# jlvdb/yet_another_wizz

Hardware: AMD Instinct MI355X
Metric: candidate pairs/s (higher is better)
Workload: dtype f64

## Files before the change

### yet_another_wizz_amd/csrc/yawhip.hip

```cpp

#include <hip/hip_runtime.h>

#include <algorithm>
#include <atomic>
#include <numeric>
#include <thread>
#include <chrono>
#include <climits>
#include <cmath>
#include <cstdarg>
#include <cstdio>
#include <cstdlib>
#include <cstring>
#include <memory>
#include <new>
#include <string>
#include <system_error>
#include <type_traits>
#include <utility>
#include <functional>
#include <vector>

#include "yawhip.h"
#include "yawhip_sort.h"

namespace {
struct Trace {
    bool on = getenv("YAWHIP_TRACE") != nullptr;
    int n = 0;
    const char *name[32];
    std::chrono::steady_clock::time_point at[32];
    void mark(const char *what) {
        if (on && n < 32) { name[n] = what; at[n++] = std::chrono::steady_clock::now(); }
    }
    void flush() {
        if (on && n > 1) {
            fprintf(stderr, "[yawhip trace]");
            for (int i = 1; i < n; ++i)
                fprintf(stderr, " %s +%.1f", name[i], std::chrono::duration<double, std::micro>(at[i] - at[i - 1]).count());
            fprintf(stderr, " | total %.1f us\n", std::chrono::duration<double, std::micro>(at[n - 1] - at[0]).count());
        }
        n = 0;
    }
};
thread_local Trace g_trace;


constexpr int WG = 256;
constexpr int STAGE = 256;
#ifndef YAW_MSTAGE
#define YAW_MSTAGE 64
#endif
#ifndef YAW_MWG
#define YAW_MWG 64
#endif
constexpr int MWG = YAW_MWG;
static_assert(MWG == 64, "the band kernels are single-wave workgroups: their lane tile is 64 * R objects");
constexpr int MSTAGE = YAW_MSTAGE;
constexpr int MAX_EDGES = 512;
constexpr int SEG_STRIPS_MIN_RUN = 16;
constexpr int BAND_MIN_STREAM_RUN = 64;
constexpr int64_t SYNC_GRID_MIN_ITEMS = 400000;
constexpr int MAX_STRIP_REACH = 12;
constexpr int COUNT_FLUSH_MASK = (1 << 13) - 1;
constexpr int MERGED_FLUSH_MASK = (1 << 16) - 1;
constexpr int SPLIT_JOBS = 1;
constexpr double PAD_COORD = 4.0;

thread_local std::string g_last_error;

int fail(int code, const char *fmt, ...) {
    char buf[1024];
    va_list ap;
    va_start(ap, fmt);
    vsnprintf(buf, sizeof buf, fmt, ap);
    va_end(ap);
    g_last_error = buf;
    return code;
}

#define HIP_TRY(expr)                                                                              \
    do {                                                                                           \
        hipError_t e_ = (expr);                                                                    \
        if (e_ != hipSuccess)                                                                      \
            return fail(e_ == hipErrorOutOfMemory ? YAWHIP_ERR_OOM : YAWHIP_ERR_HIP, "%s failed: %s (%s:%d)", \
                        #expr, hipGetErrorString(e_), __FILE__, __LINE__);                         \
    } while (0)

struct CatView {
    const double *x, *y, *z, *w;
    const int64_t *off;
    int nb;
    const double *key;
    int axis;
};

struct alignas(16) Obj {
    double x, y, z, w;
};

struct alignas(16) ObjF {
    float x, y, z, pad;
};

constexpr double FILTER_GUARD = 8.0 * 5.9604644775390625e-8;
constexpr double UNIT_NORM_TOL = 1e-9;

constexpr int MAX_WIN = 3;
struct alignas(16) Item {
    int64_t a0;
    int32_t na;
    int32_t slot;
    int32_t pot;
    int32_t nwin;
    int64_t b0[MAX_WIN];
    int32_t nb[MAX_WIN];
    int32_t pad_;
};
static_assert(sizeof(Item) == 64, "Item layout");
constexpr int SLOT_MASK = 0x3fffffff;
__host__ __device__ inline int item_slot(const Item &it) { return it.slot & SLOT_MASK; }
__host__ __device__ inline int item_orient(const Item &it) { return (int)((unsigned)it.slot >> 30); }

typedef const __attribute__((address_space(1))) double *gf64p;
typedef const __attribute__((address_space(1))) int32_t *gi32p;
typedef const __attribute__((address_space(1))) int64_t *gi64p;
#ifndef YAW_B32_PREFETCH
#define YAW_B32_PREFETCH 0
#endif
#ifndef YAW_B32_UNROLL
#define YAW_B32_UNROLL 1
#endif
#ifndef YAW_B32_PAIRS
#define YAW_B32_PAIRS 1
#endif
#ifndef YAW_B32_SHARE
#define YAW_B32_SHARE 1
#endif
#define YAW_STR_(x) #x
#define YAW_STR(x) YAW_STR_(x)
#ifndef YAW_B32_ITEM_PREFETCH
#define YAW_B32_ITEM_PREFETCH 0
#endif
#ifndef YAW_B32_AW_EARLY
#define YAW_B32_AW_EARLY 1
#endif
#ifndef YAW_B32_WAVES_W
#define YAW_B32_WAVES_W 5
#endif
#ifndef YAW_B32_WAVES_W1
#define YAW_B32_WAVES_W1 5
#endif
#ifndef YAW_B32_WAVES_BIG
#define YAW_B32_WAVES_BIG 6
#endif
#ifndef YAW_B32_WAVES_LT
#define YAW_B32_WAVES_LT 1
#endif
#ifndef YAW_B32_WAVES
#define YAW_B32_WAVES 1
#endif
typedef float f32x2 __attribute__((ext_vector_type(2)));
typedef float f32x4 __attribute__((ext_vector_type(4)));
typedef const __attribute__((address_space(1))) float *gf32p;
struct DevTab {
    gf64p x, y, z, w;
    gi32p k;
    gi64p off;
    gi64p vbase, slo, tiles;
    const struct TileRec *tile_rec;
    const struct RunGrid *grid;
    gf32p qx, qy, qz;
    gi32p idx;
    gi32p pos3;
    int32_t axis;
    int32_t pad_;
};
__device__ __forceinline__ gf64p tab_key(const DevTab &t) { return t.axis == 0 ? t.x : (t.axis == 1 ? t.y : t.z); }

struct TileRec {
    int64_t a0;
    int32_t na;
    int32_t run;
};
struct JobRec {
    int64_t t_lo;
    int64_t k_off;
    int64_t vbase1;
    int32_t n_strips1;
    int32_t o;
};
#ifndef YAW_RUN_GRID
#define YAW_RUN_GRID 64
#endif
#ifndef YAW_BUILD_BISECT
#define YAW_BUILD_BISECT 32
#endif
constexpr int RUN_GRID = YAW_RUN_GRID;
struct RunGrid {
    double inv;
    uint32_t g[RUN_GRID + 2];
};
__device__ __forceinline__ int run_cell(double key, double first, double inv) {
    const double f = (key - first) * inv;
    return f >= (double)RUN_GRID ? RUN_GRID - 1 : (f >= 1.0 ? (int)f : 0);
}
template <typename KeyT>
__global__ __launch_bounds__(256) void k_run_grid(int64_t n_runs, const int64_t *__restrict__ off, const KeyT *__restrict__ key,
                                                  RunGrid *__restrict__ grid) {
    const int64_t i = (int64_t)blockIdx.x * blockDim.x + threadIdx.x;
    const int64_t r = i / (RUN_GRID + 1);
    const int c = (int)(i - r * (RUN_GRID + 1));
    if (r >= n_runs) return;
    const int64_t b0 = off[r], b1 = off[r + 1];
    double inv = 0.0, first = 0.0;
    if (b1 > b0) {
        first = (double)key[b0];
        const double span = (double)key[b1 - 1] - first;
        inv = span > 0.0 ? (double)RUN_GRID / span : 0.0;
        if (!(inv < 1e300)) inv = 0.0;
    }
    int64_t l = b0, h = b1;
    while (l < h) {
        const int64_t m = (l + h) >> 1;
        if (run_cell((double)key[m], first, inv) < c) l = m + 1; else h = m;
    }
    grid[r].g[c] = (uint32_t)(l - b0);
    if (c == 0) { grid[r].inv = inv; grid[r].g[RUN_GRID + 1] = 0; }
}

__global__ __launch_bounds__(256) void k_merge_triples(int64_t n, int64_t n_runs, const int64_t *__restrict__ off,
                                                       const int32_t *__restrict__ run_group, const int64_t *__restrict__ vbase,
                                                       const int64_t *__restrict__ off3, const double *__restrict__ key,
                                                       const float *__restrict__ q, int64_t q_stride, const double *__restrict__ w,
                                                       float *__restrict__ q3, int64_t q3_stride, double *__restrict__ w3,
                                                       int32_t *__restrict__ idx3, int32_t *__restrict__ pos3) {
    const int64_t i = (int64_t)blockIdx.x * blockDim.x + threadIdx.x;
    if (i >= n) return;
    int64_t lo = 0, hi = n_runs;
    while (hi - lo > 1) {
        const int64_t mid = (lo + hi) >> 1;
        if (off[mid] <= i) lo = mid; else hi = mid;
    }
    const int64_t r = lo;
    const int64_t g = run_group[r], g_lo = vbase[g], g_hi = vbase[g + 1];
    const double ki = key[i];
    const float fx = q[i], fy = q[q_stride + i], fz = q[2 * q_stride + i];
    const double wi = w ? w[i] : 0.0;
    int64_t before[5];
#pragma unroll
    for (int d = -2; d <= 2; ++d) {
        const int64_t m = r + d;
        int64_t cnt = 0;
        if (d == 0) {
            cnt = i - off[r];
        } else if (m >= g_lo && m < g_hi) {
            int64_t l = off[m], h = off[m + 1];
            const int64_t base = l;
            if (d < 0) { while (l < h) { const int64_t mid = (l + h) >> 1; if (key[mid] <= ki) l = mid + 1; else h = mid; } }
            else       { while (l < h) { const int64_t mid = (l + h) >> 1; if (key[mid] < ki) l = mid + 1; else h = mid; } }
            cnt = l - base;
        }
        before[d + 2] = cnt;
    }
#pragma unroll
    for (int d = -1; d <= 1; ++d) {
        const int64_t t = r + d + 1 + 2 * g;
        const int64_t dst = off3[t] + before[d + 1] + before[d + 2] + before[d + 3];
        q3[dst] = fx; q3[q3_stride + dst] = fy; q3[2 * q3_stride + dst] = fz;
        idx3[dst] = (int32_t)i;
        if (w3) w3[dst] = wi;
        if (d == 0) pos3[i] = (int32_t)dst;
    }
}

constexpr int EVAL_SLOTS = 256;
constexpr int BUILD_WG = 1024;
#ifndef YAW_BUILD_WG_SMALL
#define YAW_BUILD_WG_SMALL 256
#endif
inline int build_wg_for(int64_t n_pot) { return n_pot / 256 <= 4096 ? YAW_BUILD_WG_SMALL : BUILD_WG; }
constexpr int BUILD_PREFIX_LDS = 1024;

constexpr int ITEM_SEGS = 8;
__host__ __device__ constexpr int ITEM_SEG_CTR(int seg) { return 12 + 8 * seg; }
__device__ __forceinline__ void append_items(bool keep, const Item &it, unsigned long long work, Item *__restrict__ items,
                                             unsigned long long *__restrict__ counters, unsigned char *__restrict__ kept,
                                             unsigned long long seg_cap = 0) {
    if (keep && kept) kept[it.pot] = 1;
    __shared__ unsigned int s_cnt[BUILD_WG / 64];
    __shared__ unsigned long long s_work[BUILD_WG / 64], s_base;
    const unsigned long long mask = __builtin_amdgcn_ballot_w64(keep);
    const int lane = threadIdx.x & 63, wave = threadIdx.x >> 6;
    for (int off = 32; off > 0; off >>= 1) work += __shfl_down(work, off, 64);
    if (lane == 0) {
        s_cnt[wave] = (unsigned int)__popcll(mask);
        s_work[wave] = work;
    }
    __syncthreads();
    if (threadIdx.x == 0) {
        unsigned int total = 0;
        unsigned long long wsum = 0;
        for (int wv = 0; wv < (int)(blockDim.x >> 6); ++wv) {
            const unsigned int c = s_cnt[wv];
            s_cnt[wv] = total;
            total += c;
            wsum += s_work[wv];
        }
        if (seg_cap) {
            const int seg = (int)(blockIdx.x % ITEM_SEGS);
            s_base = (unsigned long long)seg * seg_cap + (total ? atomicAdd(&counters[ITEM_SEG_CTR(seg)], (unsigned long long)total) : 0ull);
        } else {
            s_base = total ? atomicAdd(&counters[0], (unsigned long long)total) : 0ull;
        }
        if (wsum) atomicAdd(&counters[10 + 8 * (blockIdx.x & (EVAL_SLOTS - 1))], wsum);
    }
    __syncthreads();
    if (keep) items[s_base + s_cnt[wave] + __popcll(mask & ((1ull << lane) - 1ull))] = it;
}

template <bool SWEEP>
__global__ __launch_bounds__(BUILD_WG) void k_build_items(CatView c1, CatView c2, const int32_t *__restrict__ jobs,
                                                     const int64_t *__restrict__ prefix, int n_slots, int n_bins,
                                                     int tile, const double *__restrict__ rwin, int64_t n_pot,
                                                     Item *__restrict__ items, unsigned long long *__restrict__ counters,
                                                     unsigned char *__restrict__ kept) {
    const int64_t pot = (int64_t)blockIdx.x * blockDim.x + threadIdx.x;
    bool keep = false;
    Item it{};
    unsigned long long work = 0;
    if (pot < n_pot) {
        int lo = 0, hi = n_slots;
        while (hi - lo > 1) {
            const int mid = (lo + hi) >> 1;
            if (prefix[mid] <= pot) lo = mid; else hi = mid;
        }
        const int slot = lo, job = slot / n_bins, k = slot - job * n_bins;
        const int p = jobs[2 * job], q = jobs[2 * job + 1];
        const int k1 = c1.nb == 1 ? 0 : k, k2 = c2.nb == 1 ? 0 : k;
        int64_t b0 = c1.off[(int64_t)p * c1.nb + k1], b1 = c1.off[(int64_t)p * c1.nb + k1 + 1];
        const int64_t a_seg1 = c2.off[(int64_t)q * c2.nb + k2 + 1];
        const int64_t a0 = c2.off[(int64_t)q * c2.nb + k2] + (pot - prefix[slot]) * (int64_t)tile;
        const int64_t a1 = a0 + tile < a_seg1 ? a0 + tile : a_seg1;
        if (SWEEP) {
            const double wlo = c2.key[a0] - rwin[k], whi = c2.key[a1 - 1] + rwin[k];
            int64_t l = b0, h = b1;
            while (l < h) {
                const int64_t m = (l + h) >> 1;
                if (c1.key[m] < wlo) l = m + 1; else h = m;
            }
            const int64_t first = l;
            h = b1;
            while (l < h) {
                const int64_t m = (l + h) >> 1;
                if (c1.key[m] <= whi) l = m + 1; else h = m;
            }
            b0 = first;
            b1 = l;
        }
        keep = b1 > b0;
        it.a0 = a0; it.b0[0] = b0; it.na = (int32_t)(a1 - a0); it.nb[0] = (int32_t)(b1 - b0); it.nwin = 1; it.slot = slot; it.pot = (int32_t)pot;
        work = keep ? (unsigned long long)it.na * (unsigned long long)it.nb[0] : 0ull;
    }
    if (SWEEP) {
        append_items(keep, it, work, items, counters, kept);
    } else {
        if (pot < n_pot) items[pot] = it;
        append_items(false, it, work, items, counters, nullptr);
        if (pot == 0) counters[0] = (unsigned long long)n_pot;
    }
}

__global__ __launch_bounds__(BUILD_WG) void k_build_items_strips(const DevTab *__restrict__ tabs, const JobRec *__restrict__ jobs,
                                                            const int64_t *__restrict__ prefix, int n_jobs, int reach,
                                                            int tile, double rwin, int swap, int triple, int64_t n_pot,
                                                            Item *__restrict__ items, unsigned long long *__restrict__ counters,
                                                            unsigned char *__restrict__ kept, unsigned long long seg_cap) {
    const int64_t pot = (int64_t)blockIdx.x * blockDim.x + threadIdx.x;
    bool keep = false;
    Item it{};
    unsigned long long work = 0;
    __shared__ int64_t s_prefix[BUILD_PREFIX_LDS];
    __shared__ DevTab s_tabs[6];
    static_assert(sizeof(DevTab) % 8 == 0, "DevTab is copied in 8-byte words");
    for (int e = threadIdx.x; e < (int)(6 * sizeof(DevTab) / 8); e += blockDim.x)
        reinterpret_cast<uint64_t *>(s_tabs)[e] = reinterpret_cast<const uint64_t *>(tabs)[e];
    const bool prefix_in_lds = n_jobs + 1 <= BUILD_PREFIX_LDS;
    if (prefix_in_lds)
        for (int e = threadIdx.x; e <= n_jobs; e += blockDim.x) s_prefix[e] = prefix[e];
    __syncthreads();
    if (pot < n_pot) {
        int lo = 0, hi = n_jobs;
        if (prefix_in_lds) {
            while (hi - lo > 1) {
                const int mid = (lo + hi) >> 1;
                if (s_prefix[mid] <= pot) lo = mid; else hi = mid;
            }
        } else {
            while (hi - lo > 1) {
                const int mid = (lo + hi) >> 1;
                if (prefix[mid] <= pot) lo = mid; else hi = mid;
            }
        }
        const int job = lo;
        const JobRec jr = jobs[job];
        const int o = jr.o & 3;
        it.pad_ = (jr.o >> 2) & 1;
#if defined(YAW_BUILD_TABS_GLOBAL)
        const DevTab &c1 = tabs[swap ? 3 + o : o], &c2 = tabs[swap ? o : 3 + o];
#else
        const DevTab &c1 = s_tabs[swap ? 3 + o : o], &c2 = s_tabs[swap ? o : 3 + o];
#endif
        const gf64p key1d = tab_key(c1), key2 = tab_key(c2);
        const gf32p key1f = c1.axis == 0 ? c1.qx : (c1.axis == 1 ? c1.qy : c1.qz);
        auto key1 = [&](int64_t i) { return triple ? (double)key1f[i] : key1d[i]; };
        const int nd = 2 * reach + 1, ng = (nd + MAX_WIN - 1) / MAX_WIN;
        const int64_t local = pot - (prefix_in_lds ? s_prefix[job] : prefix[job]);
        const uint32_t local32 = (uint32_t)local, tl = ng == 1 ? local32 : local32 / (uint32_t)ng;
        const int g = (int)(local32 - tl * (uint32_t)ng);
        const TileRec tr = c2.tile_rec[jr.t_lo + tl];
        const int64_t r2 = tr.run, a0 = tr.a0, a1 = a0 + tr.na;
        const double kpad = triple ? 1.2e-7 : 0.0;
        const double wlo = key2[a0] - (it.pad_ ? 0.0 : rwin) - kpad, whi = key2[a1 - 1] + rwin + kpad;
        it.a0 = a0; it.na = tr.na; it.nwin = 0;
        it.slot = (int32_t)((unsigned)job | ((unsigned)o << 30)); it.pot = (int32_t)pot;
        int64_t wb[MAX_WIN];
        uint32_t sl[MAX_WIN], sh[MAX_WIN], ul[MAX_WIN], uh[MAX_WIN];
        int32_t wn[MAX_WIN];
#pragma unroll
        for (int j = 0; j < MAX_WIN; ++j) {
            const int dd = g * MAX_WIN + j;
            const int64_t s1 = r2 + jr.k_off + (dd - reach);
            const bool valid = dd < nd && s1 >= 0 && s1 < jr.n_strips1;
            const int64_t r1 = jr.vbase1 + (valid ? s1 : 0);
            int64_t b0 = 0, b1 = 0;
            if (valid) { b0 = c1.off[r1]; b1 = c1.off[r1 + 1]; }
            const bool some = b1 > b0;
            double kfirst = 0.0, klast = 0.0;
            if (some) { kfirst = key1(b0); klast = key1(b1 - 1); }
            const bool live = some && !(klast < wlo || kfirst > whi);
            uint32_t l0 = 0, l1 = 0, u0 = 0, u1 = 0;
            if (live) {
                const double inv = c1.grid[r1].inv;
                const int cl = run_cell(wlo, kfirst, inv), cu = run_cell(whi, kfirst, inv);
                const uint32_t *gr = c1.grid[r1].g;
                l0 = gr[cl]; l1 = gr[cl + 1]; u0 = gr[cu]; u1 = gr[cu + 1];
            }
            wb[j] = b0;
            sl[j] = l0; sh[j] = l1; ul[j] = u0; uh[j] = u1;
        }
        for (int step = 0; step < YAW_BUILD_BISECT &&
                           ((sl[0] < sh[0]) | (sl[1] < sh[1]) | (sl[2] < sh[2]) | (ul[0] < uh[0]) | (ul[1] < uh[1]) | (ul[2] < uh[2])); ++step) {
            double kl[MAX_WIN], ku[MAX_WIN];
            uint32_t ml[MAX_WIN], mu[MAX_WIN];
#pragma unroll
            for (int j = 0; j < MAX_WIN; ++j) {
                ml[j] = sl[j] + ((sh[j] - sl[j]) >> 1);
                mu[j] = ul[j] + ((uh[j] - ul[j]) >> 1);
                kl[j] = ku[j] = 0.0;
                if (sl[j] < sh[j]) kl[j] = key1(wb[j] + ml[j]);
                if (ul[j] < uh[j]) ku[j] = key1(wb[j] + mu[j]);
            }
#pragma unroll
            for (int j = 0; j < MAX_WIN; ++j) {
                if (sl[j] < sh[j]) { if (kl[j] < wlo) sl[j] = ml[j] + 1; else sh[j] = ml[j]; }
                if (ul[j] < uh[j]) { if (ku[j] <= whi) ul[j] = mu[j] + 1; else uh[j] = mu[j]; }
            }
        }
#pragma unroll
        for (int j = 0; j < MAX_WIN; ++j) {
            wb[j] += sl[j];
            wn[j] = (int32_t)((YAW_BUILD_BISECT < 32 ? uh[j] : ul[j]) - sl[j]);
        }
#pragma unroll
        for (int j = 0; j < MAX_WIN; ++j) {
            if (wn[j] <= 0) continue;
            if (it.nwin == 0) { it.b0[0] = wb[j]; it.nb[0] = wn[j]; }
            else if (it.nwin == 1) { it.b0[1] = wb[j]; it.nb[1] = wn[j]; }
            else { it.b0[2] = wb[j]; it.nb[2] = wn[j]; }
            ++it.nwin;
            work += (unsigned long long)it.na * (unsigned long long)wn[j];
// ... 1026 lines not shown
            const unsigned ic = have ? (unsigned)(lane * R + r) : 0u;
            ax[r] = have ? (cl.qx + it.a0)[ic] : PAD_COORD32;
            ay[r] = have ? (cl.qy + it.a0)[ic] : PAD_COORD32;
            az[r] = have ? (cl.qz + it.a0)[ic] : PAD_COORD32;
            kb[r] = MERGED ? (have ? (cl.k + it.a0)[ic] : 0) : 0;
            aw[r] = (WEIGHTED && cl.w) ? (have ? (cl.w + it.a0)[ic] : 0.0) : (have ? 1.0 : 0.0);
        }
        float klo, khi;
        {
            const int last_r = n_own > 0 ? n_own - 1 : 0;
            float u_first = cl.axis == 0 ? ax[0] : (cl.axis == 1 ? ay[0] : az[0]), u_last = u_first;
#pragma unroll
            for (int r = 1; r < R; ++r)
                if (r == last_r) u_last = cl.axis == 0 ? ax[r] : (cl.axis == 1 ? ay[r] : az[r]);
            klo = u_first - rwin;
            khi = u_last + rwin;
        }
        unsigned int nev = 0;
        auto flush_counts = [&]() {
#if defined(YAW_FINE_DIAG) && YAW_FINE_DIAG == 5
            return;
#endif
            __syncthreads();
            for (int idx = lane; idx < nslots; idx += 64) {
                const unsigned int c = (unsigned int)hist[idx];
                hist[idx] = HistT(0);
                if (c) atomicAdd(&out_counts[(int64_t)islot * nslots + idx], (unsigned long long)c);
            }
        };
        float pm[R], pa[R];
        unsigned a_edges[R], a_rowh[R];
        const float nf_f = (float)nf;
        const unsigned a_stab = (unsigned)(size_t)(lds_byte *)reinterpret_cast<unsigned char *>(stab);
#pragma unroll
        for (int r = 0; r < R; ++r) {
            const int trow = (UNI ? 0 : (MERGED ? kb[r] : kfix)) * tw;
            pm[r] = stab[trow]; pa[r] = stab[trow + 1];
            a_edges[r] = a_stab + (unsigned)(trow + 4) * 4u;
            a_rowh[r] = a_hist + ((unsigned)(kb[r] * nf) << HB);
        }
        f32x2 ax2[R / 2 > 0 ? R / 2 : 1], ay2[R / 2 > 0 ? R / 2 : 1], az2[R / 2 > 0 ? R / 2 : 1];
        if constexpr (R >= 2) {
#pragma unroll
            for (int h = 0; h < R / 2; ++h) {
                ax2[h] = f32x2{ax[2 * h], ax[2 * h + 1]}; ay2[h] = f32x2{ay[2 * h], ay[2 * h + 1]}; az2[h] = f32x2{az[2 * h], az[2 * h + 1]};
            }
        }

        for (int win = 0; win < it.nwin; ++win) {
        if (win > 0) {
            b0 = win == 1 ? it.b0[1] : it.b0[2];
            nb_total = win == 1 ? it.nb[1] : it.nb[2];
        }
        for (int64_t st0 = 0; st0 < nb_total; st0 += CAP, ++stage_no) {
            const int n = (int)(nb_total - st0 < CAP ? nb_total - st0 : CAP);
            if (st0 > 0 || win > 0) {
                __syncthreads();
                stage_in(st0, n);
            }
            asm volatile("s_waitcnt vmcnt(0)" ::: "memory");
            __syncthreads();
            if (lane == 0) {
                stage[n] = PAD_COORD32; stage[COLB / 4 + n] = PAD_COORD32; stage[2 * (COLB / 4) + n] = PAD_COORD32;
                if (WEIGHTED) sw[n] = 0.0;
            }
            if (WEIGHTED && !cs.w)
                for (int e = lane; e < n; e += 64) sw[e] = 1.0;
            __syncthreads();
            const unsigned a_key = a_stage + COLB * (unsigned)cl.axis;
            const unsigned a_sent = a_key + ((unsigned)n << 2);
            unsigned ql = a_key - 4u, qh = ql;
            for (unsigned step = 4u << (31 - __builtin_clz(n)); step >= 4u; step >>= 1) {
                const unsigned pl = ql + step, ph = qh + step;
                const float kl = *(const __attribute__((address_space(3))) float *)(size_t)(pl < a_sent ? pl : a_sent);
                const float kh = *(const __attribute__((address_space(3))) float *)(size_t)(ph < a_sent ? ph : a_sent);
                ql = kl < klo ? pl : ql;
                qh = kh <= khi ? ph : qh;
            }
            int lo = (int)((ql + 4u - a_key) >> 2), hi = (int)((qh + 4u - a_key) >> 2);
            if (n_own == 0) lo = hi = n;
            const int len = hi - lo;
            nev += (unsigned int)(len * n_own);
#if defined(YAW_FINE_DIAG) && YAW_FINE_DIAG == 1
            const int steps = 0;
#else
            const int steps = wave_max_nonneg(len);
#endif

            unsigned cur = a_stage + ((unsigned)lo << 2);
            const unsigned last = a_stage + ((unsigned)n << 2);
            struct Entry { float x, y, z; double w; unsigned at; };
            auto fetch = [&](unsigned at) {
                Entry e;
                e.at = at < last ? at : last;
                e.x = *(const __attribute__((address_space(3))) float *)(size_t)e.at;
                e.y = *(const __attribute__((address_space(3))) float *)(size_t)(e.at + COLB);
                e.z = *(const __attribute__((address_space(3))) float *)(size_t)(e.at + 2 * COLB);
                e.w = WEIGHTED ? lds_f64(((e.at - a_stage) << 1) + a_sw) : 1.0;
                return e;
            };
            unsigned pend[R];
#pragma unroll
            for (int r = 0; r < R; ++r) pend[r] = a_dummy;
            Entry nxt = fetch(cur);
            if constexpr (WEIGHTED) asm volatile("" :: "v"(nxt.x), "v"(nxt.y), "v"(nxt.z), "v"(nxt.w));
            else asm volatile("" :: "v"(nxt.x), "v"(nxt.y), "v"(nxt.z));
            for (int s = 0; s < steps; ++s) {
                const Entry en = nxt;
                cur += 4;
                nxt = fetch(cur);
                const unsigned a16 = en.at;
                const float ex = en.x, ey = en.y, ez = en.z;
                const double ew = en.w;
                float s32[R];
                if constexpr (R >= 2) {
#pragma unroll
                    for (int h = 0; h < R / 2; ++h) {
                        const f32x2 dx = ax2[h] - ex, dy = ay2[h] - ey, dz = az2[h] - ez;
                        const f32x2 sq = __builtin_elementwise_fma(dz, dz, __builtin_elementwise_fma(dy, dy, dx * dx));
                        s32[2 * h] = sq.x; s32[2 * h + 1] = sq.y;
                    }
                } else {
                    const float dx = ax[0] - ex, dy = ay[0] - ey, dz = az[0] - ez;
                    s32[0] = __builtin_fmaf(dz, dz, __builtin_fmaf(dy, dy, dx * dx));
                }
                int jj[R];
                bool unc[R];
                unsigned long long any_unc_mask = 0ull;
                f32x2 tb[R];
#pragma unroll
                for (int r = 0; r < R; ++r) {
                    const float fr = __builtin_rintf(__builtin_fmaf(__builtin_amdgcn_logf(s32[r]), pm[r], -pa[r]));
                    jj[r] = (int)__builtin_amdgcn_fmed3f(fr, 0.0f, nf_f);
                    tb[r] = *(const __attribute__((address_space(3))) f32x2 *)(size_t)(a_edges[r] + ((unsigned)jj[r] << 3));
                }
                if constexpr (!WEIGHTED) {
#pragma unroll
                    for (int r = 0; r < R; ++r)
                        (void)__hip_atomic_fetch_add((__attribute__((address_space(3))) unsigned int *)(size_t)pend[r], 1u,
                                                     __ATOMIC_RELAXED, __HIP_MEMORY_SCOPE_WORKGROUP);
                }
#pragma unroll
                for (int r = 0; r < R; ++r) {
                    const int j = jj[r];
                    const bool below = s32[r] < tb[r].x, above = s32[r] > tb[r].y;
                    const int bin = j - (below ? 1 : 0);
                    unc[r] = !(below | above);
                    any_unc_mask |= ~(__builtin_amdgcn_ballot_w64(below) | __builtin_amdgcn_ballot_w64(above));
                    const bool hit = ((unsigned)bin < (unsigned)nf) & !unc[r];
                    const unsigned cell = a_rowh[r] + ((unsigned)bin << HB);
                    if constexpr (WEIGHTED) {
                        if (hit)
                            (void)__hip_atomic_fetch_add((__attribute__((address_space(3))) double *)(size_t)cell, aw[r] * ew,
                                                         __ATOMIC_RELAXED, __HIP_MEMORY_SCOPE_WORKGROUP);
                    } else {
                        pend[r] = hit ? cell : a_dummy;
                    }
                }
#if defined(YAW_FINE_DIAG) && YAW_FINE_DIAG == 6
                any_unc_mask = 0ull;
#endif
                if (any_unc_mask != 0ull) {
                    const unsigned eidx = (a16 - a_stage) >> 2;
#pragma unroll
                    for (int r = 0; r < R; ++r) {
                        if (unc[r] && eidx < (unsigned)n && r < n_own) {
                            const int j = jj[r];
                            const ExactEval<1> ev = band32_exact<1>(cl.x, cl.y, cl.z, it.a0 + lane * R + r, cs.x, cs.y, cs.z,
                                                                    cs.idx ? (int64_t)cs.idx[b0 + st0 + eidx] : b0 + st0 + (int64_t)eidx,
                                                                    t + (size_t)(MERGED ? kb[r] : kfix) * n_edges + j,
                                                                    counters + 9 + 8 * (ticket & (EVAL_SLOTS - 1)));
                            const int bin = ev.s <= ev.th[0] ? j - 1 : j;
                            if ((unsigned)bin < (unsigned)nf) {
                                const unsigned cell = a_rowh[r] + ((unsigned)bin << HB);
                                if constexpr (WEIGHTED)
                                    (void)__hip_atomic_fetch_add((__attribute__((address_space(3))) double *)(size_t)cell, aw[r] * ew,
                                                                 __ATOMIC_RELAXED, __HIP_MEMORY_SCOPE_WORKGROUP);
                                else
                                    (void)__hip_atomic_fetch_add((__attribute__((address_space(3))) unsigned int *)(size_t)cell, 1u,
                                                                 __ATOMIC_RELAXED, __HIP_MEMORY_SCOPE_WORKGROUP);
                            }
                        }
                    }
                }
            }
            if constexpr (!WEIGHTED) {
#pragma unroll
                for (int r = 0; r < R; ++r)
                    (void)__hip_atomic_fetch_add((__attribute__((address_space(3))) unsigned int *)(size_t)pend[r], 1u,
                                                 __ATOMIC_RELAXED, __HIP_MEMORY_SCOPE_WORKGROUP);
            }
            if (!WEIGHTED && (stage_no & flush_mask) == flush_mask) flush_counts();
        }
        }
        if constexpr (WEIGHTED) {
            __syncthreads();
            for (int idx = lane; idx < nslots; idx += 64) {
                partials[(int64_t)it.pot * nslots + idx] = (double)hist[idx];
                hist[idx] = HistT(0);
            }
        } else {
            flush_counts();
        }
        nev = wave_sum_lane63(nev);
        if (lane == 63 && nev) atomicAdd(&counters[8 + 8 * (ticket & (EVAL_SLOTS - 1))], (unsigned long long)nev);
    }
}

__global__ void k_item_work(const Item *__restrict__ items, const unsigned long long *__restrict__ counters,
                            int slots_per_job, unsigned long long *__restrict__ job_work) {
    const unsigned long long i = (unsigned long long)blockIdx.x * blockDim.x + threadIdx.x;
    if (i >= counters[0]) return;
    const Item it = items[i];
    unsigned long long streamed = 0;
    for (int w = 0; w < it.nwin; ++w) streamed += (unsigned long long)it.nb[w];
    atomicAdd(&job_work[item_slot(it) / slots_per_job], (unsigned long long)it.na * streamed);
}

constexpr int REDUCE_CHUNK = 32;
__global__ void k_reduce_chunks(const double *__restrict__ partials, const unsigned char *__restrict__ kept,
                                const int64_t *__restrict__ prefix, const int64_t *__restrict__ cprefix, int n_slots,
                                int slab, double *__restrict__ chunk_sums) {
    const int64_t idx = (int64_t)blockIdx.x * blockDim.x + threadIdx.x;
    const int64_t g = idx / slab;
    if (g >= cprefix[n_slots]) return;
    const int e = (int)(idx - g * slab);
    int lo = 0, hi = n_slots;
    while (hi - lo > 1) {
        const int mid = (lo + hi) >> 1;
        if (cprefix[mid] <= g) lo = mid; else hi = mid;
    }
    const int64_t p0 = prefix[lo] + (g - cprefix[lo]) * REDUCE_CHUNK;
    const int64_t p1 = p0 + REDUCE_CHUNK < prefix[lo + 1] ? p0 + REDUCE_CHUNK : prefix[lo + 1];
    double acc = 0.0;
    for (int64_t pot = p0; pot < p1; ++pot)
        if (!kept || kept[pot]) acc += partials[pot * slab + e];
    chunk_sums[idx] = acc;
}

__global__ void k_reduce_slots(const double *__restrict__ chunk_sums, const int64_t *__restrict__ cprefix, int n_slots,
                               int slab, double *__restrict__ out) {
    const int64_t idx = (int64_t)blockIdx.x * blockDim.x + threadIdx.x;
    if (idx >= (int64_t)n_slots * slab) return;
    const int slot = (int)(idx / slab), e = (int)(idx - (int64_t)slot * slab);
    double acc = 0.0;
    for (int64_t g = cprefix[slot]; g < cprefix[slot + 1]; ++g) acc += chunk_sums[g * slab + e];
    out[idx] = acc;
}

template <typename F>
__device__ double numpy_sum_dev(F v, int lo, int n) {
    if (n < 8) {
        double res = 0.0;
        for (int i = 0; i < n; ++i) res += v(lo + i);
        return res;
    }
    if (n <= 128) {
        double r[8];
        for (int j = 0; j < 8; ++j) r[j] = v(lo + j);
        int i = 8;
        for (; i < n - (n % 8); i += 8)
            for (int j = 0; j < 8; ++j) r[j] += v(lo + i + j);
        double res = ((r[0] + r[1]) + (r[2] + r[3])) + ((r[4] + r[5]) + (r[6] + r[7]));
        for (; i < n; ++i) res += v(lo + i);
        return res;
    }
    int n2 = n / 2;
    n2 -= n2 % 8;
    return numpy_sum_dev(v, lo, n2) + numpy_sum_dev(v, lo + n2, n - n2);
}

__global__ void k_combine_scales(const unsigned long long *__restrict__ counts, const double *__restrict__ sums, int weighted,
                                 int64_t n_jobs, int n_bins, int nf, int n_scales, const int32_t *__restrict__ slices,
                                 const double *__restrict__ factors, double *__restrict__ out) {
    const int64_t i = (int64_t)blockIdx.x * blockDim.x + threadIdx.x;
    if (i >= n_jobs * n_bins * n_scales) return;
    const int sc = (int)(i % n_scales), k = (int)((i / n_scales) % n_bins);
    const int64_t j = i / ((int64_t)n_scales * n_bins);
    const int lo = slices[2 * (k * n_scales + sc)], hi = slices[2 * (k * n_scales + sc) + 1];
    const int64_t base = (j * n_bins + k) * (int64_t)nf;
    const double *wk = factors ? factors + (int64_t)k * nf : nullptr;
    auto value = [&](int e) {
        const double v = weighted ? sums[base + e] : (double)counts[base + e];
        return wk ? v * wk[e] : v;
    };
    out[i] = hi > lo ? numpy_sum_dev(value, lo, hi - lo) : 0.0;
}

__global__ void k_scatter_rows(const double *__restrict__ in, const int32_t *__restrict__ row_index, int64_t row, int64_t n,
                               double *__restrict__ out) {
    const int64_t i = (int64_t)blockIdx.x * blockDim.x + threadIdx.x;
    if (i >= n) return;
    const int64_t r = i / row;
    out[(int64_t)row_index[r] * row + (i - r * row)] = in[i];
}

__global__ void k_counts_to_double(const unsigned long long *__restrict__ in, double *__restrict__ out, int64_t n) {
    const int64_t i = (int64_t)blockIdx.x * blockDim.x + threadIdx.x;
    if (i < n) out[i] = (double)in[i];
}

inline DevTab make_tab(const double *x, const double *y, const double *z, const double *w, const int32_t *k, const int64_t *off,
                       const int64_t *vbase, const int64_t *slo, const int64_t *tiles, const TileRec *tile_rec, const RunGrid *grid,
                       int axis, const float *q = nullptr, int64_t q_stride = 0, const int32_t *idx = nullptr) {
    return DevTab{(gf64p)x, (gf64p)y, (gf64p)z, (gf64p)w, (gi32p)k, (gi64p)off, (gi64p)vbase, (gi64p)slo, (gi64p)tiles,
                  tile_rec, grid, (gf32p)q, (gf32p)(q ? q + q_stride : nullptr), (gf32p)(q ? q + 2 * q_stride : nullptr), (gi32p)idx,
                  (gi32p)nullptr, axis, 0};
}

template <typename T>
struct DevBuf {
    T *ptr = nullptr;
    size_t cap = 0;
    hipError_t reserve(size_t n) {
        if (n <= cap) return hipSuccess;
        if (ptr) (void)hipFree(ptr);
        ptr = nullptr;
        cap = 0;
        size_t want = n + n / 4 + 64;
        hipError_t e = hipMalloc(reinterpret_cast<void **>(&ptr), want * sizeof(T));
        if (e == hipSuccess) cap = want;
        return e;
    }
    void release() {
        if (ptr) (void)hipFree(ptr);
        ptr = nullptr;
        cap = 0;
    }
};

struct Arena {
    unsigned char *h = nullptr, *d = nullptr;
    size_t cap = 0;
    hipError_t reserve(size_t n) {
        if (n <= cap) return hipSuccess;
        release();
        const size_t want = n + n / 4 + 4096;
        hipError_t e = hipHostMalloc(reinterpret_cast<void **>(&h), want, hipHostMallocPortable);
        if (e == hipSuccess) e = hipMalloc(reinterpret_cast<void **>(&d), want);
        if (e == hipSuccess) cap = want; else release();
        return e;
    }
    void release() {
        if (h) (void)hipHostFree(h);
        if (d) (void)hipFree(d);
        h = d = nullptr;
        cap = 0;
    }
};
inline size_t align16(size_t n) { return (n + 15) & ~(size_t)15; }

}

template <typename T>
struct View {
    T *ptr = nullptr;
};

struct CallBufs {
    hipEvent_t ev0 = nullptr, ev1 = nullptr, evc0 = nullptr, evc1 = nullptr, ev_done = nullptr;
    View<int32_t> d_jobs;
    View<int64_t> d_prefix;
    View<double> d_t;
    View<float> d_dthr;
    View<float> d_thr32;
    View<double> d_rwin;
    DevBuf<Item> d_items;
    View<unsigned long long> d_ctr;
    View<unsigned long long> d_counts;
    View<double> d_sums;
    DevBuf<double> d_partials;
    DevBuf<double> d_chunk_sums;
    View<int64_t> d_cprefix;
    DevBuf<unsigned char> d_kept;
    Arena out;
    Arena comb;
    View<DevTab> d_tabs;
    hipError_t make_events() {
        hipError_t e = hipSuccess;
        for (hipEvent_t *ev : {&ev0, &ev1, &evc0, &evc1, &ev_done})
            if (e == hipSuccess && !*ev) e = hipEventCreate(ev);
        return e;
    }
    void release_all() {
        d_items.release(); d_partials.release(); d_chunk_sums.release(); d_kept.release();
        out.release(); comb.release();
        for (hipEvent_t *ev : {&ev0, &ev1, &evc0, &evc1, &ev_done}) {
            if (*ev) (void)hipEventDestroy(*ev);
            *ev = nullptr;
        }
    }
};
constexpr int MAX_BATCH = 4;
constexpr size_t MAX_PLANS = 16;

namespace {
struct HostPlan;

struct CallKey {
    uint64_t c1_uid = 0, c2_uid = 0, opt_gen = 0, hash = 0;
    int32_t n_jobs = 0, n_bins = 0, n_edges = 0, kernel = 0, n_dev = 0;
    bool want_counts = false, want_sums = false, for_work = false;
    const int32_t *jobs = nullptr;
    const double *t = nullptr;
    std::vector<int32_t> own_jobs;
    std::vector<double> own_t;

    CallKey() = default;
    CallKey(const yawhip_ctx *ctx, const yawhip_catalog *c1, const yawhip_catalog *c2, int32_t n_jobs, const int32_t *jobs,
            int32_t n_bins, int32_t n_edges, const double *t, int32_t kernel, bool want_counts, bool want_sums, bool for_work,
            int32_t n_dev = 0);
    CallKey(CallKey &&) = default;
    CallKey &operator=(CallKey &&) = default;
    CallKey(const CallKey &) = delete;
    CallKey &operator=(const CallKey &) = delete;

    void keep() {
        own_jobs.assign(jobs, jobs + 2 * (size_t)n_jobs);
        own_t.assign(t, t + (size_t)n_bins * n_edges);
        jobs = own_jobs.data();
        t = own_t.data();
    }
    bool operator==(const CallKey &o) const {
        return hash == o.hash && c1_uid == o.c1_uid && c2_uid == o.c2_uid && opt_gen == o.opt_gen && n_jobs == o.n_jobs &&
               n_bins == o.n_bins && n_edges == o.n_edges && kernel == o.kernel && n_dev == o.n_dev && want_counts == o.want_counts &&
               want_sums == o.want_sums && for_work == o.for_work &&
               memcmp(jobs, o.jobs, sizeof(int32_t) * 2 * (size_t)n_jobs) == 0 &&
               memcmp(t, o.t, sizeof(double) * (size_t)n_bins * n_edges) == 0;
    }
};
}

struct yawhip_ctx : CallBufs {
    int device = 0;
    hipStream_t stream = nullptr;
    int tile_r = 0;
    int hist_copies_log2 = -1;
    int band_batch_log2 = -1;
    int band_cap = 0;
    int seg_strips = 1;
    int seg_min_run = SEG_STRIPS_MIN_RUN;
    int debug_no_hits = 0;
    int auto_orient = 1;
    int64_t slab_budget = 1ll << 30;
    int band_grid_div = 0;
    int flush_log2 = 17;
    int spin_wait = 1;
    int item_segments = 1;
    int half_bands = 1;
    int triple_runs = 1;
    int band_fp32 = 1;
    double strip_width = 0.005;
    int default_kernel = YAWHIP_KERNEL_AUTO;
    int lds_limit = 160 * 1024;
    int n_cu = 256;
    DevBuf<unsigned long long> d_jobwork;
    DevBuf<double> d_full;
    DevBuf<int32_t> d_rowidx;
    std::vector<yawhip_ctx *> peers;
    struct Plan {
        CallKey key;
        std::vector<std::vector<int32_t>> parts;
    } plan;
    yawsort::Workspace sort_ws;
    CallBufs parked[MAX_BATCH];
    int slot = 0;
    uint64_t opt_gen = 1;
    uint64_t plan_clock = 0;
    std::vector<HostPlan *> plans;
};
inline hipError_t use_slot(yawhip_ctx *ctx, int i) {
    if (i != ctx->slot) {
        std::swap(static_cast<CallBufs &>(*ctx), ctx->parked[ctx->slot]);
        std::swap(static_cast<CallBufs &>(*ctx), ctx->parked[i]);
        ctx->slot = i;
    }
    return ctx->make_events();
}


struct StripLayout {
    bool built = false;
    double *x = nullptr, *y = nullptr, *z = nullptr, *w = nullptr;
    int32_t *k = nullptr;
    float *q = nullptr;
    int64_t q_stride = 0;
    int64_t *off = nullptr;
    std::vector<int64_t> h_off;
    std::vector<int64_t> h_vbase;
    std::vector<int64_t> h_slo;
    std::vector<int64_t> h_tiles[3];
    int64_t *d_vbase = nullptr, *d_slo = nullptr, *d_tiles[3] = {nullptr, nullptr, nullptr};
    TileRec *d_tile_rec[3] = {nullptr, nullptr, nullptr};
    RunGrid *d_grid = nullptr;
    bool triples = false;
    float *q3 = nullptr;
    int64_t q3_stride = 0;
    double *w3 = nullptr;
    int32_t *idx3 = nullptr;
    int32_t *pos3 = nullptr;
    int64_t *off3 = nullptr;
    RunGrid *d_grid3 = nullptr;
    int64_t n_groups = 0;
    int64_t device_bytes = 0;
    double obj_run = 0.0;
    double same_bin = 0.0;
    void release() {
        for (void *ptr : {(void *)x, (void *)y, (void *)z, (void *)w, (void *)k, (void *)q, (void *)off, (void *)d_vbase, (void *)d_slo,
                          (void *)d_tiles[0], (void *)d_tiles[1], (void *)d_tiles[2], (void *)d_tile_rec[0], (void *)d_tile_rec[1],
                          (void *)d_tile_rec[2], (void *)d_grid, (void *)q3, (void *)w3, (void *)idx3, (void *)pos3, (void *)off3, (void *)d_grid3})
            if (ptr) (void)hipFree(ptr);
        q3 = nullptr; w3 = nullptr; idx3 = nullptr; pos3 = nullptr; off3 = nullptr; d_grid3 = nullptr; triples = false;
        x = y = z = w = nullptr; k = nullptr; q = nullptr; off = d_vbase = d_slo = nullptr;
        d_tiles[0] = d_tiles[1] = d_tiles[2] = nullptr;
        d_tile_rec[0] = d_tile_rec[1] = d_tile_rec[2] = nullptr;
        d_grid = nullptr;
        built = false;
    }
};

struct yawhip_catalog {
    yawhip_ctx *ctx = nullptr;
    uint64_t uid = 0;
    int64_t n = 0;
    int32_t n_patches = 0, nb = 1;
    double *x = nullptr, *y = nullptr, *z = nullptr, *w = nullptr;
    int64_t *off = nullptr;
    std::vector<int64_t> h_off;
    int64_t device_bytes = 0;
    bool unit_norm = true;
    int axis = 2;
    StripLayout strips[3], seg[3];
    std::vector<yawhip_catalog *> replicas;
    bool has_strips = false;
    double strip_width = 0.0;
    std::vector<double> h_box;
};

namespace {

void drop_plans(yawhip_ctx *ctx, const yawhip_catalog *c);

const double *key_of(const double *x, const double *y, const double *z, int axis) { return axis == 0 ? x : (axis == 1 ? y : z); }
CatView view_of(const yawhip_catalog *c) {
    return CatView{c->x, c->y, c->z, c->w, c->off, c->nb, key_of(c->x, c->y, c->z, c->axis), c->axis};
}

template <typename... Params, typename... Args>
hipError_t launch(void (*kern)(Params...), dim3 grid, dim3 block, size_t lds, hipStream_t stream, Args... args) {
    if (lds > 64 * 1024) {
        const hipError_t e = hipFuncSetAttribute(reinterpret_cast<const void *>(kern), hipFuncAttributeMaxDynamicSharedMemorySize, (int)lds);
        if (e != hipSuccess) return e;
    }
    hipLaunchKernelGGL(kern, grid, block, lds, stream, args...);
    return hipGetLastError();
}

template <typename... Ts, typename V, typename F>
hipError_t pick(const V &v, F &&f) {
    hipError_t e = hipErrorInvalidValue;
    (void)(((v == Ts::value) && (e = f(Ts{}), true)) || ...);
    return e;
}
template <bool B> using Bool = std::integral_constant<bool, B>;
template <int I> using Int = std::integral_constant<int, I>;
template <int R_, int CAP_> struct Stage {
    static constexpr int R = R_, CAP = CAP_;
    static constexpr std::pair<int, int> value{R_, CAP_};
};
template <bool MERGED_, bool UNI_> struct Rows {
    static constexpr bool MERGED = MERGED_, UNI = UNI_;
    static constexpr std::pair<bool, bool> value{MERGED_, UNI_};
};

__global__ __launch_bounds__(256) void k_assign_patches(int64_t n, const double *__restrict__ x, const double *__restrict__ y,
                                                       const double *__restrict__ z, int n_centers,
                                                       const double *__restrict__ centers, int32_t *__restrict__ out) {
    extern __shared__ __attribute__((aligned(16))) unsigned char lds_raw[];
    double *c = reinterpret_cast<double *>(lds_raw);
    for (int e = threadIdx.x; e < 3 * n_centers; e += blockDim.x) c[e] = centers[e];
    __syncthreads();
    const int64_t i = (int64_t)blockIdx.x * blockDim.x + threadIdx.x;
    if (i >= n) return;
    const double px = x[i], py = y[i], pz = z[i];
    double best = INFINITY;
    int best_j = -1;
    for (int j = 0; j < n_centers; ++j) {
        const double dx = px - c[3 * j], dy = py - c[3 * j + 1], dz = pz - c[3 * j + 2];
        const double xx = dx * dx;
        const double yy = dy * dy;
        const double zz = dz * dz;
        const double sxy = xx + yy;
        const double d = sxy + zz;
        if (d < best) {
            best = d;
            best_j = j;
        }
    }
    out[i] = best_j;
}

__global__ void k_gather_columns(int64_t n, const uint32_t *__restrict__ perm, const double *__restrict__ sx,
                                 const double *__restrict__ sy, const double *__restrict__ sz, const double *__restrict__ sw,
                                 double *__restrict__ dx, double *__restrict__ dy, double *__restrict__ dz, double *__restrict__ dw) {
    const int64_t i = (int64_t)blockIdx.x * blockDim.x + threadIdx.x;
    if (i >= n) return;
    const uint32_t src = perm[i];
    dx[i] = sx[src];
    dy[i] = sy[src];
    dz[i] = sz[src];
    if (sw) dw[i] = sw[src];
}

__device__ __forceinline__ int segment_of(const int64_t *__restrict__ off, int n_seg, int64_t i) {
    int lo = 0, hi = n_seg;
    while (hi - lo > 1) {
        const int mid = (lo + hi) >> 1;
        if (off[mid] <= i) lo = mid; else hi = mid;
    }
    return lo;
}

__global__ void k_gather_bins(int64_t n, const uint32_t *__restrict__ perm, const int64_t *__restrict__ off, int64_t n_seg,
                              int n_bins, int32_t *__restrict__ bins) {
    const int64_t i = (int64_t)blockIdx.x * blockDim.x + threadIdx.x;
    if (i < n) bins[i] = segment_of(off, (int)n_seg, (int64_t)perm[i]) % n_bins;
}

__global__ void k_make_q(int64_t n, const double *__restrict__ x, const double *__restrict__ y, const double *__restrict__ z,
                         int64_t stride, float *__restrict__ q) {
    const int64_t i = (int64_t)blockIdx.x * blockDim.x + threadIdx.x;
    if (i >= n) return;
    q[i] = (float)x[i];
    q[stride + i] = (float)y[i];
    q[2 * stride + i] = (float)z[i];
}

__global__ void k_same_bin_neighbours(int64_t n, const int32_t *__restrict__ bins, unsigned long long *__restrict__ out) {
    const int64_t i = (int64_t)blockIdx.x * blockDim.x + threadIdx.x;
    const bool same = i + 1 < n && bins[i] == bins[i + 1];
    const unsigned long long m = __builtin_amdgcn_ballot_w64(same);
    if ((threadIdx.x & 63) == 0 && m) atomicAdd(out, (unsigned long long)__popcll(m));
}

__global__ void k_strip_index(int64_t n, const double *__restrict__ v, double width, const int64_t *__restrict__ poff,
                              int n_patches, int32_t *__restrict__ gidx, int32_t *__restrict__ lohi) {
    const int64_t i = (int64_t)blockIdx.x * blockDim.x + threadIdx.x;
    const bool ok = i < n;
    int32_t g = 0;
    int p = -1;
    if (ok) {
        g = width > 0.0 ? (int32_t)floor((v[i] + 1.0) / width) : 0;
        gidx[i] = g;
        p = segment_of(poff, n_patches, i);
    }
    const int p0 = __builtin_amdgcn_readfirstlane(p);
    if (__builtin_amdgcn_ballot_w64(p != p0) == 0ull) {
        if (p0 < 0) return;
        int32_t lo = g, hi = g;
        for (int off = 32; off > 0; off >>= 1) {
            lo = min(lo, __shfl_xor(lo, off, 64));
            hi = max(hi, __shfl_xor(hi, off, 64));
        }
        if ((threadIdx.x & 63) == 0) {
            atomicMin(&lohi[2 * p0], lo);
            atomicMax(&lohi[2 * p0 + 1], hi);
        }
    } else if (ok) {
        atomicMin(&lohi[2 * p], g);
        atomicMax(&lohi[2 * p + 1], g);
    }
}

__global__ void k_run_of(int64_t n, const uint32_t *__restrict__ order, const int32_t *__restrict__ gidx,
                         const int64_t *__restrict__ poff, int n_patches, const int64_t *__restrict__ vbase,
                         const int64_t *__restrict__ slo, uint32_t *__restrict__ run) {
    const int64_t i = (int64_t)blockIdx.x * blockDim.x + threadIdx.x;
    if (i >= n) return;
    const uint32_t src = order[i];
    const int p = segment_of(poff, n_patches, (int64_t)src);
    run[i] = (uint32_t)(vbase[p] + (int64_t)gidx[src] - slo[p]);
}

__global__ void k_run_offsets(const uint32_t *__restrict__ run_sorted, int64_t n, int64_t n_runs, int64_t *__restrict__ moff) {
    const int64_t r = (int64_t)blockIdx.x * blockDim.x + threadIdx.x;
    if (r > n_runs) return;
    int64_t lo = 0, hi = n;
    while (lo < hi) {
        const int64_t mid = (lo + hi) >> 1;
        if ((int64_t)run_sorted[mid] < r) lo = mid + 1; else hi = mid;
    }
    moff[r] = lo;
}

__host__ __device__ inline unsigned long long sortable_of(double d) {
    unsigned long long b;
    memcpy(&b, &d, sizeof b);
    return (b >> 63) ? ~b : (b | 0x8000000000000000ull);
}
inline double double_of(unsigned long long s) {
    const unsigned long long b = (s >> 63) ? (s & 0x7fffffffffffffffull) : ~s;
    double d;
    memcpy(&d, &b, sizeof d);
    return d;
}

__global__ void k_patch_boxes(int64_t n, const double *__restrict__ x, const double *__restrict__ y, const double *__restrict__ z,
                              const int64_t *__restrict__ poff, int n_patches, unsigned long long *__restrict__ box) {
    const int64_t i = (int64_t)blockIdx.x * blockDim.x + threadIdx.x;
    const bool ok = i < n;
    double v[3] = {0.0, 0.0, 0.0};
    int p = -1;
    bool off_sphere = false;
    if (ok) {
        v[0] = x[i]; v[1] = y[i]; v[2] = z[i];
        p = segment_of(poff, n_patches, i);
        const double n2 = v[0] * v[0] + v[1] * v[1] + v[2] * v[2];
        off_sphere = !(n2 > 1.0 - UNIT_NORM_TOL && n2 < 1.0 + UNIT_NORM_TOL);
    }
    if (__builtin_amdgcn_ballot_w64(off_sphere) != 0ull && (threadIdx.x & 63) == 0) atomicAdd(&box[(size_t)6 * n_patches], 1ull);
    const int p0 = __builtin_amdgcn_readfirstlane(p);
    if (__builtin_amdgcn_ballot_w64(p != p0) == 0ull) {
        if (p0 < 0) return;
#pragma unroll
        for (int a = 0; a < 3; ++a) {
            unsigned long long lo = sortable_of(v[a]), hi = lo;
            for (int off = 32; off > 0; off >>= 1) {
                const unsigned long long l2 = __shfl_xor(lo, off, 64), h2 = __shfl_xor(hi, off, 64);
                lo = l2 < lo ? l2 : lo;
                hi = h2 > hi ? h2 : hi;
            }
            if ((threadIdx.x & 63) == 0) {
                atomicMin(&box[(size_t)6 * p0 + a], lo);
                atomicMax(&box[(size_t)6 * p0 + 3 + a], hi);
            }
        }
    } else if (ok) {
#pragma unroll
        for (int a = 0; a < 3; ++a) {
            atomicMin(&box[(size_t)6 * p + a], sortable_of(v[a]));
            atomicMax(&box[(size_t)6 * p + 3 + a], sortable_of(v[a]));
        }
    }
}

inline int64_t seg_len(const yawhip_catalog *c, int patch, int k) {
    const int kk = c->nb == 1 ? 0 : k;
    const int64_t i = (int64_t)patch * c->nb + kk;
    return c->h_off[i + 1] - c->h_off[i];
}

int build_strip_layout(yawhip_ctx *ctx, yawhip_catalog *c, int o, bool seg) {
    StripLayout &L = seg ? c->seg[o] : c->strips[o];
    if (L.built) return YAWHIP_OK;
    const int64_t n = c->n, nseg = (int64_t)c->n_patches * c->nb;
    const int n_groups = seg ? (int)nseg : c->n_patches;
    const bool want_bins = !seg && c->nb > 1;
    const double width = c->strip_width;
    const int saxis = (o + 2) % 3;
    std::vector<int64_t> h_poff((size_t)n_groups + 1);
    for (int g = 0; g <= n_groups; ++g) h_poff[(size_t)g] = seg ? c->h_off[(size_t)g] : c->h_off[(size_t)g * c->nb];
    const size_t col = (size_t)std::max<int64_t>(n, 1) * sizeof(double) + 16;
    uint32_t *perm = nullptr, *perm2 = nullptr, *run = nullptr, *run_sorted = nullptr;
    int32_t *gidx = nullptr, *lohi = nullptr;
    int64_t *poff = nullptr;
    auto bail = [&](hipError_t err, const char *what) {
        for (void *q : {(void *)perm, (void *)perm2, (void *)run, (void *)run_sorted, (void *)gidx, (void *)lohi, (void *)poff})
            if (q) (void)hipFree(q);
        if (err == hipSuccess) return (int)YAWHIP_OK;
        L.release();
        return fail(err == hipErrorOutOfMemory ? YAWHIP_ERR_OOM : YAWHIP_ERR_HIP, "strip layout (%s) failed: %s", what,
                    hipGetErrorString(err));
    };
    HIP_TRY(hipSetDevice(ctx->device));
    std::vector<int32_t> h_lohi((size_t)2 * n_groups);
    for (int g = 0; g < n_groups; ++g) { h_lohi[(size_t)2 * g] = INT32_MAX; h_lohi[(size_t)2 * g + 1] = INT32_MIN; }
    const size_t n1 = (size_t)std::max<int64_t>(n, 1);
    hipError_t e = hipMalloc(reinterpret_cast<void **>(&poff), (size_t)(n_groups + 1) * sizeof(int64_t));
    if (e == hipSuccess) e = hipMalloc(reinterpret_cast<void **>(&lohi), (size_t)2 * n_groups * sizeof(int32_t));
    if (e == hipSuccess) e = hipMalloc(reinterpret_cast<void **>(&gidx), n1 * sizeof(int32_t));
    if (e == hipSuccess) e = hipMalloc(reinterpret_cast<void **>(&perm), n1 * sizeof(uint32_t));
    if (e == hipSuccess) e = hipMalloc(reinterpret_cast<void **>(&perm2), n1 * sizeof(uint32_t));
    if (e == hipSuccess) e = hipMalloc(reinterpret_cast<void **>(&run), n1 * sizeof(uint32_t));
    if (e == hipSuccess) e = hipMalloc(reinterpret_cast<void **>(&run_sorted), n1 * sizeof(uint32_t));
    if (e == hipSuccess)
        e = hipMemcpyAsync(poff, h_poff.data(), (size_t)(n_groups + 1) * sizeof(int64_t), hipMemcpyHostToDevice, ctx->stream);
    if (e == hipSuccess)
        e = hipMemcpyAsync(lohi, h_lohi.data(), (size_t)2 * n_groups * sizeof(int32_t), hipMemcpyHostToDevice, ctx->stream);
    if (e != hipSuccess) return bail(e, "strip tables");
    const unsigned ngrid = (unsigned)((n1 + 255) / 256);
    hipLaunchKernelGGL(k_strip_index, dim3(ngrid), dim3(256), 0, ctx->stream, n, key_of(c->x, c->y, c->z, saxis), width, poff,
                       n_groups, gidx, lohi);
    e = hipMemcpyAsync(h_lohi.data(), lohi, (size_t)2 * n_groups * sizeof(int32_t), hipMemcpyDeviceToHost, ctx->stream);
    if (e == hipSuccess) e = hipStreamSynchronize(ctx->stream);
    if (e != hipSuccess) return bail(e, "strip index");
    std::vector<int64_t> vbase((size_t)n_groups + 1, 0), slo((size_t)n_groups, 0);
    for (int g = 0; g < n_groups; ++g) {
        const bool any = h_poff[(size_t)g + 1] > h_poff[(size_t)g];
        slo[(size_t)g] = any ? h_lohi[(size_t)2 * g] : 0;
        vbase[(size_t)g + 1] = vbase[(size_t)g] + (any ? (int64_t)h_lohi[(size_t)2 * g + 1] - h_lohi[(size_t)2 * g] + 1 : 0);
    }
    const int64_t n_runs = vbase[(size_t)n_groups];
    if (n_runs >= (1ll << 31)) return bail(hipErrorInvalidValue, "too many strip runs");
    int run_bits = 1;
    while ((1ll << run_bits) < n_runs) ++run_bits;
    e = hipMalloc(reinterpret_cast<void **>(&L.d_vbase), (size_t)(n_groups + 1) * sizeof(int64_t));
    if (e == hipSuccess) e = hipMalloc(reinterpret_cast<void **>(&L.d_slo), (size_t)std::max(n_groups, 1) * sizeof(int64_t));
    if (e == hipSuccess)
        e = hipMemcpyAsync(L.d_vbase, vbase.data(), (size_t)(n_groups + 1) * sizeof(int64_t), hipMemcpyHostToDevice, ctx->stream);
    if (e == hipSuccess)
        e = hipMemcpyAsync(L.d_slo, slo.data(), (size_t)n_groups * sizeof(int64_t), hipMemcpyHostToDevice, ctx->stream);
    if (e == hipSuccess) e = yawsort::sort_segments(ctx->sort_ws, ctx->stream, n, key_of(c->x, c->y, c->z, o), poff, n_groups, perm);
    if (e != hipSuccess) return bail(e, "group sort");
    hipLaunchKernelGGL(k_run_of, dim3(ngrid), dim3(256), 0, ctx->stream, n, perm, gidx, poff, n_groups, L.d_vbase, L.d_slo, run);
    e = yawsort::sort_runs(ctx->sort_ws, ctx->stream, n, run, perm, run_bits, perm2, run_sorted);
    if (e != hipSuccess) return bail(e, "run sort");
    e = hipMalloc(reinterpret_cast<void **>(&L.x), col);
    if (e == hipSuccess) e = hipMalloc(reinterpret_cast<void **>(&L.y), col);
    if (e == hipSuccess) e = hipMalloc(reinterpret_cast<void **>(&L.z), col);
    if (e == hipSuccess && c->w) e = hipMalloc(reinterpret_cast<void **>(&L.w), col);
    if (e == hipSuccess && want_bins) e = hipMalloc(reinterpret_cast<void **>(&L.k), n1 * sizeof(int32_t) + 16);
    L.q_stride = (int64_t)((n1 + 3) & ~(size_t)3) + 8;
    if (e == hipSuccess) e = hipMalloc(reinterpret_cast<void **>(&L.q), (size_t)3 * L.q_stride * sizeof(float));
    if (e == hipSuccess) e = hipMalloc(reinterpret_cast<void **>(&L.off), (size_t)(n_runs + 1) * sizeof(int64_t));
    if (e == hipSuccess) e = hipMalloc(reinterpret_cast<void **>(&L.d_grid), (size_t)(n_runs + 1) * sizeof(RunGrid));
    if (e == hipSuccess) e = hipMemsetAsync(L.d_grid, 0, (size_t)(n_runs + 1) * sizeof(RunGrid), ctx->stream);
    if (e != hipSuccess) return bail(e, "strip layout");
    hipLaunchKernelGGL(k_gather_columns, dim3(ngrid), dim3(256), 0, ctx->stream, n, perm2, c->x, c->y, c->z, c->w, L.x, L.y, L.z, L.w);
    if (want_bins)
        hipLaunchKernelGGL(k_gather_bins, dim3(ngrid), dim3(256), 0, ctx->stream, n, perm2, c->off, nseg, c->nb, L.k);
    hipLaunchKernelGGL(k_make_q, dim3(ngrid), dim3(256), 0, ctx->stream, n, L.x, L.y, L.z, L.q_stride, L.q);
    hipLaunchKernelGGL(k_run_offsets, dim3((unsigned)((n_runs + 1 + 255) / 256)), dim3(256), 0, ctx->stream, run_sorted, n, n_runs,
                       L.off);
    if (n_runs > 0)
        hipLaunchKernelGGL(k_run_grid<double>, dim3((unsigned)((n_runs * (RUN_GRID + 1) + 255) / 256)), dim3(256), 0, ctx->stream, n_runs,
                           L.off, o == 0 ? L.x : (o == 1 ? L.y : L.z), L.d_grid);
    std::vector<int64_t> voff((size_t)n_runs + 1);
    e = hipMemcpyAsync(voff.data(), L.off, (size_t)(n_runs + 1) * sizeof(int64_t), hipMemcpyDeviceToHost, ctx->stream);
    unsigned long long h_same = 0;
    if (want_bins && n > 1) {
        unsigned long long *d_same = reinterpret_cast<unsigned long long *>(run);
        if (e == hipSuccess) e = hipMemsetAsync(d_same, 0, sizeof(unsigned long long), ctx->stream);
        if (e == hipSuccess) {
            hipLaunchKernelGGL(k_same_bin_neighbours, dim3(ngrid), dim3(256), 0, ctx->stream, n, L.k, d_same);
            e = hipMemcpyAsync(&h_same, d_same, sizeof(unsigned long long), hipMemcpyDeviceToHost, ctx->stream);
        }
    }
    if (e == hipSuccess) e = hipStreamSynchronize(ctx->stream);
    if (e != hipSuccess) return bail(e, "run offsets");
    L.same_bin = n > 1 ? (double)h_same / (double)(n - 1) : 0.0;
    for (int64_t r = 0; r < n_runs; ++r)
        if (voff[(size_t)r + 1] - voff[(size_t)r] >= (1ll << 32)) return bail(hipErrorInvalidValue, "a strip run of 2^32 objects or more");
    for (int ri = 0; ri < 3; ++ri) {
        const int64_t tile = (int64_t)MWG << ri;
        L.h_tiles[ri].assign((size_t)n_runs + 1, 0);
        for (int64_t r = 0; r < n_runs; ++r)
            L.h_tiles[ri][(size_t)r + 1] = L.h_tiles[ri][(size_t)r] + (voff[(size_t)r + 1] - voff[(size_t)r] + tile - 1) / tile;
        {
            const int64_t n_tiles = L.h_tiles[ri][(size_t)n_runs];
            std::vector<TileRec> tile_rec((size_t)std::max<int64_t>(n_tiles, 1), TileRec{0, 0, 0});
            for (int64_t r = 0; r < n_runs; ++r)
                for (int64_t tl = L.h_tiles[ri][(size_t)r]; tl < L.h_tiles[ri][(size_t)r + 1]; ++tl) {
                    const int64_t a0 = voff[(size_t)r] + (tl - L.h_tiles[ri][(size_t)r]) * tile;
                    tile_rec[(size_t)tl] = TileRec{a0, (int32_t)std::min<int64_t>(tile, voff[(size_t)r + 1] - a0), (int32_t)r};
                }
            if (e == hipSuccess) e = hipMalloc(reinterpret_cast<void **>(&L.d_tile_rec[ri]), tile_rec.size() * sizeof(TileRec));
            if (e == hipSuccess)
                e = hipMemcpy(L.d_tile_rec[ri], tile_rec.data(), tile_rec.size() * sizeof(TileRec), hipMemcpyHostToDevice);
        }
        if (e == hipSuccess) e = hipMalloc(reinterpret_cast<void **>(&L.d_tiles[ri]), (size_t)(n_runs + 1) * sizeof(int64_t));
        if (e == hipSuccess)
            e = hipMemcpyAsync(L.d_tiles[ri], L.h_tiles[ri].data(), (size_t)(n_runs + 1) * sizeof(int64_t),
                               hipMemcpyHostToDevice, ctx->stream);
    }
    if (e == hipSuccess) e = hipStreamSynchronize(ctx->stream);
    if (e != hipSuccess) return bail(e, "tile tables");
    {
        double sq = 0.0;
        for (int64_t r = 0; r < n_runs; ++r) {
            const double len = (double)(voff[(size_t)r + 1] - voff[(size_t)r]);
            sq += len * len;
        }
        L.obj_run = n > 0 ? sq / (double)n : 0.0;
    }
    L.h_off = std::move(voff);
    L.h_vbase = std::move(vbase);
    L.h_slo = std::move(slo);
    L.n_groups = n_groups;
    L.device_bytes = (int64_t)col * (c->w ? 4 : 3) + (want_bins ? n * (int64_t)sizeof(int32_t) : 0) + 3 * L.q_stride * (int64_t)sizeof(float) +
                     (4 * (n_runs + 1) + 2 * (int64_t)n_groups + 1) * (int64_t)sizeof(int64_t) + (n_runs + 1) * (int64_t)sizeof(RunGrid) +
                     (L.h_tiles[0][(size_t)n_runs] + L.h_tiles[1][(size_t)n_runs] + L.h_tiles[2][(size_t)n_runs]) * (int64_t)sizeof(TileRec);
    c->device_bytes += L.device_bytes;
    L.built = true;
    return bail(hipSuccess, "");
}

int build_triples(yawhip_ctx *ctx, yawhip_catalog *c, int o, bool seg) {
    StripLayout &L = seg ? c->seg[o] : c->strips[o];
    if (!L.built) return fail(YAWHIP_ERR_INVALID, "build_triples: layout not built");
    if (L.triples) return YAWHIP_OK;
    const int64_t n = c->n, G = L.n_groups, V = L.h_vbase[(size_t)G], V3 = V + 2 * G;
    if (3 * n >= (1ll << 31)) return fail(YAWHIP_ERR_INVALID, "build_triples: catalogue too large for 32-bit entry indices");
    std::vector<int64_t> off3((size_t)V3 + 1, 0);
    std::vector<int32_t> run_group((size_t)std::max<int64_t>(V, 1), 0);
    for (int64_t g = 0; g < G; ++g) {
        const int64_t lo = L.h_vbase[(size_t)g], hi = L.h_vbase[(size_t)g + 1];
        for (int64_t r = lo; r < hi; ++r) run_group[(size_t)r] = (int32_t)g;
        for (int64_t c_rel = 0; c_rel < hi - lo + 2; ++c_rel) {
            const int64_t t = lo + 2 * g + c_rel, rc = lo + c_rel - 1;
            int64_t len = 0;
            for (int64_t m = rc - 1; m <= rc + 1; ++m)
                if (m >= lo && m < hi) len += L.h_off[(size_t)m + 1] - L.h_off[(size_t)m];
            off3[(size_t)t + 1] = len;
        }
    }
    for (int64_t t = 0; t < V3; ++t) off3[(size_t)t + 1] += off3[(size_t)t];
    if (off3[(size_t)V3] != 3 * n) return fail(YAWHIP_ERR_HIP, "build_triples: %lld entries for %lld objects", (long long)off3[(size_t)V3], (long long)n);
    HIP_TRY(hipSetDevice(ctx->device));
    const size_t n3 = (size_t)std::max<int64_t>(3 * n, 1);
    L.q3_stride = (int64_t)((n3 + 3) & ~(size_t)3) + 8;
    int32_t *d_run_group = nullptr;
    hipError_t e = hipMalloc(reinterpret_cast<void **>(&L.q3), (size_t)3 * L.q3_stride * sizeof(float));
    if (e == hipSuccess) e = hipMalloc(reinterpret_cast<void **>(&L.idx3), n3 * sizeof(int32_t));
    if (e == hipSuccess) e = hipMalloc(reinterpret_cast<void **>(&L.pos3), (size_t)std::max<int64_t>(n, 1) * sizeof(int32_t));
    if (e == hipSuccess && c->w) e = hipMalloc(reinterpret_cast<void **>(&L.w3), n3 * sizeof(double) + 16);
    if (e == hipSuccess) e = hipMalloc(reinterpret_cast<void **>(&L.off3), (size_t)(V3 + 1) * sizeof(int64_t));
    if (e == hipSuccess) e = hipMalloc(reinterpret_cast<void **>(&L.d_grid3), (size_t)(V3 + 1) * sizeof(RunGrid));
    if (e == hipSuccess) e = hipMalloc(reinterpret_cast<void **>(&d_run_group), run_group.size() * sizeof(int32_t));
    if (e == hipSuccess) e = hipMemsetAsync(L.q3, 0, (size_t)3 * L.q3_stride * sizeof(float), ctx->stream);
    if (e == hipSuccess) e = hipMemsetAsync(L.d_grid3, 0, (size_t)(V3 + 1) * sizeof(RunGrid), ctx->stream);
    if (e == hipSuccess) e = hipMemcpyAsync(L.off3, off3.data(), (size_t)(V3 + 1) * sizeof(int64_t), hipMemcpyHostToDevice, ctx->stream);
    if (e == hipSuccess) e = hipMemcpyAsync(d_run_group, run_group.data(), run_group.size() * sizeof(int32_t), hipMemcpyHostToDevice, ctx->stream);
    if (e == hipSuccess && n > 0) {
        hipLaunchKernelGGL(k_merge_triples, dim3((unsigned)((n + 255) / 256)), dim3(256), 0, ctx->stream, n, V, L.off, d_run_group,
                           L.d_vbase, L.off3, o == 0 ? L.x : (o == 1 ? L.y : L.z), L.q, L.q_stride, L.w, L.q3, L.q3_stride, L.w3, L.idx3, L.pos3);
        hipLaunchKernelGGL(k_run_grid<float>, dim3((unsigned)((V3 * (RUN_GRID + 1) + 255) / 256)), dim3(256), 0, ctx->stream, V3, L.off3,
                           L.q3 + (size_t)o * L.q3_stride, L.d_grid3);
        e = hipGetLastError();
    }
    if (e == hipSuccess) e = hipStreamSynchronize(ctx->stream);
    if (d_run_group) (void)hipFree(d_run_group);
    if (e != hipSuccess) {
        for (void *ptr : {(void *)L.q3, (void *)L.w3, (void *)L.idx3, (void *)L.pos3, (void *)L.off3, (void *)L.d_grid3})
            if (ptr) (void)hipFree(ptr);
        L.q3 = nullptr; L.w3 = nullptr; L.idx3 = nullptr; L.pos3 = nullptr; L.off3 = nullptr; L.d_grid3 = nullptr;
        return fail(e == hipErrorOutOfMemory ? YAWHIP_ERR_OOM : YAWHIP_ERR_HIP, "merged triple runs failed: %s", hipGetErrorString(e));
    }
    const int64_t bytes = 3 * L.q3_stride * (int64_t)sizeof(float) + (int64_t)n3 * (4 + (c->w ? 8 : 0)) + n * 4 + (V3 + 1) * (int64_t)(sizeof(int64_t) + sizeof(RunGrid));
    L.device_bytes += bytes;
    c->device_bytes += bytes;
    L.triples = true;
    return YAWHIP_OK;
}

}

extern "C" {

const char *yawhip_last_error(void) { return g_last_error.c_str(); }
int yawhip_abi_version(void) { return YAWHIP_ABI_VERSION; }

int yawhip_device_count(int *n) {
    if (!n) return fail(YAWHIP_ERR_INVALID, "yawhip_device_count: n is NULL");
    int c = 0;
    hipError_t e = hipGetDeviceCount(&c);
    if (e != hipSuccess) {
        *n = 0;
        return fail(YAWHIP_ERR_NO_DEVICE, "hipGetDeviceCount failed: %s", hipGetErrorString(e));
    }
    *n = c;
    return YAWHIP_OK;
}

int yawhip_ctx_create(int device_id, yawhip_ctx **out) {
    if (!out) return fail(YAWHIP_ERR_INVALID, "yawhip_ctx_create: out is NULL");
    *out = nullptr;
    int c = 0;
    if (hipGetDeviceCount(&c) != hipSuccess || c <= 0)
        return fail(YAWHIP_ERR_NO_DEVICE, "no HIP device visible (the HIP path is mandatory; there is no CPU fallback)");
    if (device_id < 0 || device_id >= c)
        return fail(YAWHIP_ERR_NO_DEVICE, "device id %d out of range [0,%d)", device_id, c);
    HIP_TRY(hipSetDevice(device_id));
    yawhip_ctx *ctx = new (std::nothrow) yawhip_ctx();
    if (!ctx) return fail(YAWHIP_ERR_OOM, "host allocation failed");
    ctx->device = device_id;
    hipError_t e = hipStreamCreateWithFlags(&ctx->stream, hipStreamNonBlocking);
    if (e == hipSuccess) e = ctx->make_events();
    if (e != hipSuccess) {
        delete ctx;
        return fail(YAWHIP_ERR_HIP, "context setup failed: %s", hipGetErrorString(e));
    }
    hipDeviceProp_t prop;
    if (hipGetDeviceProperties(&prop, device_id) == hipSuccess) {
        if (prop.sharedMemPerBlock > 0) ctx->lds_limit = (int)std::min<size_t>(prop.sharedMemPerBlock, 160 * 1024);
        if (prop.multiProcessorCount > 0) ctx->n_cu = prop.multiProcessorCount;
    }
    *out = ctx;
    return YAWHIP_OK;
}

int yawhip_ctx_destroy(yawhip_ctx *ctx) {
    if (!ctx) return YAWHIP_OK;
    for (yawhip_ctx *peer : ctx->peers) (void)yawhip_ctx_destroy(peer);
    ctx->peers.clear();
    (void)hipSetDevice(ctx->device);
    if (ctx->stream) (void)hipStreamSynchronize(ctx->stream);
    drop_plans(ctx, nullptr);
    ctx->release_all();
    for (CallBufs &pb : ctx->parked) pb.release_all();
    ctx->d_jobwork.release();
    ctx->d_full.release();
    ctx->d_rowidx.release();
    ctx->sort_ws.release();
    if (ctx->stream) (void)hipStreamDestroy(ctx->stream);
    delete ctx;
    return YAWHIP_OK;
}

int yawhip_ctx_set_option(yawhip_ctx *ctx, const char *key, int64_t value) {
    if (!ctx || !key) return fail(YAWHIP_ERR_INVALID, "yawhip_ctx_set_option: NULL argument");
    std::function<void(yawhip_ctx &)> set;
    auto flag = [&](int yawhip_ctx::*field) { set = [=](yawhip_ctx &c) { c.*field = value != 0; }; };
    auto number = [&](int yawhip_ctx::*field) { set = [=](yawhip_ctx &c) { c.*field = (int)value; }; };
    if (!strcmp(key, "half_bands")) {
        flag(&yawhip_ctx::half_bands);
    } else if (!strcmp(key, "tile_r")) {
        if (value != 0 && value != 1 && value != 2 && value != 4)
            return fail(YAWHIP_ERR_INVALID, "tile_r must be 0 (auto), 1, 2 or 4");
        number(&yawhip_ctx::tile_r);
    } else if (!strcmp(key, "band_batch_log2")) {
        if (value < -1 || value > 6) return fail(YAWHIP_ERR_INVALID, "band_batch_log2 must be -1 (auto) or 0..6");
        number(&yawhip_ctx::band_batch_log2);
    } else if (!strcmp(key, "hist_copies_log2")) {
        if (value < -1 || value > 6) return fail(YAWHIP_ERR_INVALID, "hist_copies_log2 must be -1 (auto) or 0..6");
        number(&yawhip_ctx::hist_copies_log2);
    } else if (!strcmp(key, "triple_runs")) {
        if (value < 0 || value > 2) return fail(YAWHIP_ERR_INVALID, "triple_runs must be 0, 1 or 2");
        number(&yawhip_ctx::triple_runs);
    } else if (!strcmp(key, "item_segments")) {
        flag(&yawhip_ctx::item_segments);
    } else if (!strcmp(key, "spin_wait")) {
        flag(&yawhip_ctx::spin_wait);
    } else if (!strcmp(key, "band_cap")) {
        if (value != 0 && value != BCAP && value != BCAP_MID && value != B32_CAP && value != B32_CAP_BIG)
            return fail(YAWHIP_ERR_INVALID, "band_cap must be 0 (auto), 192 or 288 (float64 / fine-grid band kernels), %d or %d (float32 band kernel)",
                        B32_CAP, B32_CAP_BIG);
        number(&yawhip_ctx::band_cap);
    } else if (!strcmp(key, "strip_width_micro")) {
        if (value != 0 && (value < 1000 || value > 2000000))
            return fail(YAWHIP_ERR_INVALID, "strip_width_micro must be 0 (off) or in [1e3, 2e6]");
        set = [=](yawhip_ctx &c) { c.strip_width = (double)value * 1e-6; };
    } else if (!strcmp(key, "seg_strips_min_run")) {
        if (value < 1) return fail(YAWHIP_ERR_INVALID, "seg_strips_min_run must be >= 1");
        set = [=](yawhip_ctx &c) { c.seg_min_run = (int)std::min<int64_t>(value, INT32_MAX); };
    } else if (!strcmp(key, "seg_strips")) {
        flag(&yawhip_ctx::seg_strips);
    } else if (!strcmp(key, "debug_no_hits")) {
        flag(&yawhip_ctx::debug_no_hits);
    } else if (!strcmp(key, "auto_orient")) {
        flag(&yawhip_ctx::auto_orient);
    } else if (!strcmp(key, "slab_budget_bytes")) {
        if (value < 4096) return fail(YAWHIP_ERR_INVALID, "slab_budget_bytes must be >= 4096");
        set = [=](yawhip_ctx &c) { c.slab_budget = value; };
    } else if (!strcmp(key, "band_grid_div")) {
        if (value < 0 || value > 64) return fail(YAWHIP_ERR_INVALID, "band_grid_div must be 0 (auto) or in [1, 64]");
        number(&yawhip_ctx::band_grid_div);
    } else if (!strcmp(key, "flush_stages_log2")) {
        if (value < 0 || value > 17) return fail(YAWHIP_ERR_INVALID, "flush_stages_log2 must be in [0, 17]");
        number(&yawhip_ctx::flush_log2);
    } else if (!strcmp(key, "band_fp32")) {
        flag(&yawhip_ctx::band_fp32);
    } else if (!strcmp(key, "kernel")) {
        if (value < YAWHIP_KERNEL_AUTO || value > YAWHIP_KERNEL_BAND)
            return fail(YAWHIP_ERR_INVALID, "unknown kernel id %lld", (long long)value);
        number(&yawhip_ctx::default_kernel);
    } else {
        return fail(YAWHIP_ERR_INVALID, "unknown option '%s'", key);
    }
    std::vector<yawhip_ctx *> devices(ctx->peers);
    devices.push_back(ctx);
    for (yawhip_ctx *c : devices) {
        ++c->opt_gen;
        drop_plans(c, nullptr);
        set(*c);
    }
    return YAWHIP_OK;
}

int yawhip_catalog_upload(yawhip_ctx *ctx, int64_t n, const double *x, const double *y, const double *z,
                          const double *w, int32_t n_patches, int32_t n_bins_or_1, const int64_t *offsets,
                          yawhip_catalog **out) {
    return yawhip_catalog_upload_axis(ctx, n, x, y, z, w, n_patches, n_bins_or_1, offsets, 2, out);
}

int yawhip_catalog_sort_axis(const yawhip_catalog *cat, int32_t *axis) {
    if (!cat || !axis) return fail(YAWHIP_ERR_INVALID, "yawhip_catalog_sort_axis: NULL argument");
    *axis = cat->axis;
    return YAWHIP_OK;
}

int yawhip_catalog_upload_axis(yawhip_ctx *ctx, int64_t n, const double *x, const double *y, const double *z,
                               const double *w, int32_t n_patches, int32_t n_bins_or_1, const int64_t *offsets,
                               int32_t sort_axis, yawhip_catalog **out) {
    if (!out) return fail(YAWHIP_ERR_INVALID, "yawhip_catalog_upload: out is NULL");
    if (sort_axis < 0 || sort_axis > 2) return fail(YAWHIP_ERR_INVALID, "sort_axis must be 0 (x), 1 (y) or 2 (z)");
    *out = nullptr;
    if (!ctx) return fail(YAWHIP_ERR_INVALID, "yawhip_catalog_upload: ctx is NULL");
    if (n < 0 || n_patches <= 0 || n_bins_or_1 <= 0 || !offsets || (n > 0 && (!x || !y || !z)))
        return fail(YAWHIP_ERR_INVALID, "yawhip_catalog_upload: bad sizes or NULL columns");
    const int64_t nseg = (int64_t)n_patches * n_bins_or_1;
    if (n >= (1ll << 32)) return fail(YAWHIP_ERR_INVALID, "at most 2^32 - 1 objects per catalogue");
    if (offsets[0] != 0 || offsets[nseg] != n) return fail(YAWHIP_ERR_INVALID, "offsets must start at 0 and end at n");
    for (int64_t i = 0; i < nseg; ++i)
        if (offsets[i + 1] < offsets[i]) return fail(YAWHIP_ERR_INVALID, "offsets must be non-decreasing");
    HIP_TRY(hipSetDevice(ctx->device));
    yawhip_catalog *c = new (std::nothrow) yawhip_catalog();
    static std::atomic<uint64_t> next_uid{1};
    if (c) c->uid = next_uid.fetch_add(1);
    if (!c) return fail(YAWHIP_ERR_OOM, "host allocation failed");
    c->ctx = ctx;
    c->n = n;
    c->n_patches = n_patches;
    c->nb = n_bins_or_1;
    c->axis = sort_axis;
    c->h_off.assign(offsets, offsets + nseg + 1);
    const size_t col = (size_t)std::max<int64_t>(n, 1) * sizeof(double) + 16;
    double *rx = nullptr, *ry = nullptr, *rz = nullptr, *rw = nullptr;
    uint32_t *perm = nullptr;
    int64_t *poff = nullptr;
    unsigned long long *box = nullptr;
    auto free_tmp = [&]() {
        for (void *q : {(void *)rx, (void *)ry, (void *)rz, (void *)rw, (void *)perm, (void *)poff, (void *)box})
            if (q) (void)hipFree(q);
    };
    auto bail = [&](hipError_t err, const char *what) {
        free_tmp();
        yawhip_catalog_free(c);
        return fail(err == hipErrorOutOfMemory ? YAWHIP_ERR_OOM : YAWHIP_ERR_HIP, "catalog upload (%s) failed: %s", what,
                    hipGetErrorString(err));
    };
    std::vector<int64_t> h_poff((size_t)n_patches + 1);
    for (int p = 0; p <= n_patches; ++p) h_poff[(size_t)p] = offsets[(int64_t)p * n_bins_or_1];
    std::vector<unsigned long long> h_box((size_t)6 * n_patches + 1);
    for (int p = 0; p < n_patches; ++p)
        for (int a = 0; a < 3; ++a) {
            h_box[(size_t)6 * p + a] = sortable_of(4.0);
            h_box[(size_t)6 * p + 3 + a] = sortable_of(-4.0);
        }
    h_box[(size_t)6 * n_patches] = 0ull;
    hipError_t e = hipMalloc(reinterpret_cast<void **>(&c->x), col);
    if (e == hipSuccess) e = hipMalloc(reinterpret_cast<void **>(&c->y), col);
    if (e == hipSuccess) e = hipMalloc(reinterpret_cast<void **>(&c->z), col);
    if (e == hipSuccess && w) e = hipMalloc(reinterpret_cast<void **>(&c->w), col);
    if (e == hipSuccess) e = hipMalloc(reinterpret_cast<void **>(&c->off), (size_t)(nseg + 1) * sizeof(int64_t));
    if (e == hipSuccess) e = hipMalloc(reinterpret_cast<void **>(&rx), col);
    if (e == hipSuccess) e = hipMalloc(reinterpret_cast<void **>(&ry), col);
    if (e == hipSuccess) e = hipMalloc(reinterpret_cast<void **>(&rz), col);
    if (e == hipSuccess && w) e = hipMalloc(reinterpret_cast<void **>(&rw), col);
    if (e == hipSuccess) e = hipMalloc(reinterpret_cast<void **>(&perm), (size_t)std::max<int64_t>(n, 1) * sizeof(uint32_t));
    if (e == hipSuccess) e = hipMalloc(reinterpret_cast<void **>(&poff), (size_t)(n_patches + 1) * sizeof(int64_t));
    if (e == hipSuccess) e = hipMalloc(reinterpret_cast<void **>(&box), h_box.size() * sizeof(unsigned long long));
    if (e == hipSuccess && n > 0) {
        e = hipMemcpyAsync(rx, x, (size_t)n * sizeof(double), hipMemcpyHostToDevice, ctx->stream);
        if (e == hipSuccess) e = hipMemcpyAsync(ry, y, (size_t)n * sizeof(double), hipMemcpyHostToDevice, ctx->stream);
        if (e == hipSuccess) e = hipMemcpyAsync(rz, z, (size_t)n * sizeof(double), hipMemcpyHostToDevice, ctx->stream);
        if (e == hipSuccess && w) e = hipMemcpyAsync(rw, w, (size_t)n * sizeof(double), hipMemcpyHostToDevice, ctx->stream);
    }
    if (e == hipSuccess)
        e = hipMemcpyAsync(c->off, offsets, (size_t)(nseg + 1) * sizeof(int64_t), hipMemcpyHostToDevice, ctx->stream);
    if (e == hipSuccess)
        e = hipMemcpyAsync(poff, h_poff.data(), (size_t)(n_patches + 1) * sizeof(int64_t), hipMemcpyHostToDevice, ctx->stream);
    if (e == hipSuccess)
        e = hipMemcpyAsync(box, h_box.data(), h_box.size() * sizeof(unsigned long long), hipMemcpyHostToDevice, ctx->stream);
    if (e != hipSuccess) return bail(e, "columns");
    const unsigned ngrid = (unsigned)((std::max<int64_t>(n, 1) + 255) / 256);
    if (n > 0) {
        hipLaunchKernelGGL(k_patch_boxes, dim3(ngrid), dim3(256), 0, ctx->stream, n, rx, ry, rz, poff, n_patches, box);
        e = yawsort::sort_segments(ctx->sort_ws, ctx->stream, n, key_of(rx, ry, rz, sort_axis), c->off, nseg, perm);
        if (e != hipSuccess) return bail(e, "segment sort");
        hipLaunchKernelGGL(k_gather_columns, dim3(ngrid), dim3(256), 0, ctx->stream, n, perm, rx, ry, rz, rw, c->x, c->y, c->z, c->w);
        if ((e = hipGetLastError()) != hipSuccess) return bail(e, "gather");
        e = hipMemcpyAsync(h_box.data(), box, h_box.size() * sizeof(unsigned long long), hipMemcpyDeviceToHost, ctx->stream);
        if (e != hipSuccess) return bail(e, "patch boxes");
    }
    e = hipStreamSynchronize(ctx->stream);
    if (e != hipSuccess) return bail(e, "finish");
    free_tmp();
    c->unit_norm = h_box[(size_t)6 * n_patches] == 0ull;
    c->h_box.resize((size_t)6 * n_patches);
    for (size_t i = 0; i < c->h_box.size(); ++i) c->h_box[i] = double_of(h_box[i]);
    c->device_bytes = (int64_t)col * (w ? 4 : 3) + (nseg + 1) * (int64_t)sizeof(int64_t);
    c->strip_width = ctx->strip_width;
    c->has_strips = c->unit_norm && n > 0;
    if (c->has_strips) {
        const int rc = build_strip_layout(ctx, c, sort_axis, false);
        if (rc != YAWHIP_OK) {
            yawhip_catalog_free(c);
            return rc;
        }
    }
    if (ctx->sort_ws.cap > ((size_t)1 << 25)) ctx->sort_ws.release();
    for (yawhip_ctx *peer : ctx->peers) {
        yawhip_catalog *rep = nullptr;
        const int rc = yawhip_catalog_upload_axis(peer, n, x, y, z, w, n_patches, n_bins_or_1, offsets, sort_axis, &rep);
        if (rc != YAWHIP_OK) {
            yawhip_catalog_free(c);
            return rc;
        }
        c->replicas.push_back(rep);
    }
    *out = c;
    return YAWHIP_OK;
}

int yawhip_catalog_free(yawhip_catalog *c) {
    if (!c) return YAWHIP_OK;
    for (yawhip_catalog *rep : c->replicas) (void)yawhip_catalog_free(rep);
    c->replicas.clear();
    if (c->ctx) (void)hipSetDevice(c->ctx->device);
    if (c->ctx) {
        if (c->ctx->stream) (void)hipStreamSynchronize(c->ctx->stream);
        drop_plans(c->ctx, c);
    }
    if (c->x) (void)hipFree(c->x);
    if (c->y) (void)hipFree(c->y);
    if (c->z) (void)hipFree(c->z);
    if (c->w) (void)hipFree(c->w);
    if (c->off) (void)hipFree(c->off);
    for (int o = 0; o < 3; ++o) {
        c->strips[o].release();
        c->seg[o].release();
    }
    delete c;
    return YAWHIP_OK;
}

int yawhip_catalog_device_bytes(const yawhip_catalog *cat, int64_t *bytes) {
    if (!cat || !bytes) return fail(YAWHIP_ERR_INVALID, "yawhip_catalog_device_bytes: NULL argument");
    *bytes = cat->device_bytes;
    return YAWHIP_OK;
}

}

namespace {

struct CallState {
    std::chrono::steady_clock::time_point wall0;
    bool pending = false;
    int64_t n_out = 0;
    size_t o_ctr = 0, o_counts = 0, o_sums = 0;
    bool want_counts = false, want_sums = false, band_ran = false, run_unweighted = false, run_weighted = false;
    bool segmented = false;
    int64_t cand = 0, abytes = 0, n_pot = 0;
    int launches = 0, kernel = 0, mode = 0, n_orient = 0, band_variant = 0, merged_triples = 0;
};

std::vector<float> build_thr32(const double *t, int n_bins, int n_edges) {
    auto down = [](double v) { float f = (float)v; if ((double)f > v) f = nextafterf(f, -INFINITY); return f; };
    auto up = [](double v) { float f = (float)v; if ((double)f < v) f = nextafterf(f, INFINITY); return f; };
    auto guard = [](double te) { return BAND32_GUARD_SQRT * std::sqrt(te) + 5e-7 * te + 1e-12; };
    const int tw = thr32_width(n_edges);
    std::vector<float> out((size_t)n_bins * tw, 0.f);
    for (int k = 0; k < n_bins; ++k) {
        const double *tk = t + (size_t)k * n_edges;
        float *row = &out[(size_t)k * tw];
        if (n_edges == 2) {
            const double g0 = guard(tk[0]), g1 = guard(tk[1]);
            const float c = (float)(0.5 * (tk[0] + tk[1]));
            const double cd = (double)c;
            const double fold = 4e-7 * cd;
            const double h_in = (std::min(cd - (tk[0] + g0), (tk[1] - g1) - cd) - fold) * (1.0 - 1e-6);
            const double h_out = (std::max(cd - (tk[0] - g0), (tk[1] + g1) - cd) + fold) * (1.0 + 1e-6);
            row[0] = c;
            row[1] = h_in > 0.0 ? down(h_in) : 0.f;
            row[2] = up(std::max(h_out, 0.0));
            row[3] = 0.f;
        } else {
            for (int e = 0; e < n_edges; ++e) {
                const double g = guard(tk[e]);
                row[2 * e] = down(tk[e] - g);
                row[2 * e + 1] = up(tk[e] + g);
            }
        }
    }
    return out;
}

std::vector<float> build_fine32(const double *t, int n_bins, int n_edges) {
    auto down = [](double v) { float f = (float)v; if ((double)f > v) f = nextafterf(f, -INFINITY); return f; };
    auto up = [](double v) { float f = (float)v; if ((double)f < v) f = nextafterf(f, INFINITY); return f; };
    auto guard = [](double te) { return BAND32_GUARD_SQRT * std::sqrt(te) + 5e-7 * te + 1e-12; };
    const int tw = fine32_width(n_edges), nf = n_edges - 1;
    std::vector<float> out((size_t)n_bins * tw, 0.f);
    for (int k = 0; k < n_bins; ++k) {
        const double *tk = t + (size_t)k * n_edges;
        if (!(tk[0] > 1e-12) || !(tk[nf] > tk[0])) return {};
        const double l0 = std::log2(tk[0]), l1 = std::log2(tk[nf]);
        const double m = (double)nf / (l1 - l0), a = l0 * m;
        double dev = 0.0;
        for (int j = 0; j <= nf; ++j) {
            if (j > 0 && !(tk[j] > tk[j - 1])) return {};
            dev = std::max(dev, std::fabs((std::log2(tk[j]) - l0) * m - (double)j));
        }
        const double dev_f = m * (1e-5 + 6e-8 * 64.0) + 2.0 * 6e-8 * std::fabs(a) + 4e-5 + 6e-8 * (nf + 2);
        const double per_s = 1.05 * m / std::log(2.0);
        if (dev + dev_f + per_s * guard(tk[0]) / tk[0] > 0.45) return {};
        float *row = &out[(size_t)k * tw];
        row[0] = (float)m; row[1] = (float)a; row[2] = 0.f; row[3] = 0.f;
        for (int j = 0; j <= nf; ++j) {
            const double g = guard(tk[j]);
            row[4 + 2 * j] = down(tk[j] - g);
            row[5 + 2 * j] = up(tk[j] + g);
        }
    }
    return out;
}

CallKey::CallKey(const yawhip_ctx *ctx, const yawhip_catalog *c1, const yawhip_catalog *c2, int32_t n_jobs_, const int32_t *jobs_,
                 int32_t n_bins_, int32_t n_edges_, const double *t_, int32_t kernel_, bool want_counts_, bool want_sums_,
                 bool for_work_, int32_t n_dev_)
    : c1_uid(c1->uid), c2_uid(c2->uid), opt_gen(ctx->opt_gen), n_jobs(n_jobs_), n_bins(n_bins_), n_edges(n_edges_),
      kernel(kernel_), n_dev(n_dev_), want_counts(want_counts_), want_sums(want_sums_), for_work(for_work_), jobs(jobs_), t(t_) {
    auto mix = [this](uint64_t w) { hash = (hash ^ w) * 0x100000001b3ull; hash ^= hash >> 29; };
    for (uint64_t w : {c1_uid, c2_uid, opt_gen, (uint64_t)(uint32_t)n_jobs << 32 | (uint32_t)n_bins,
                       (uint64_t)(uint32_t)n_edges << 32 | (uint32_t)kernel,
                       (uint64_t)(uint32_t)n_dev << 32 | (uint64_t)(want_counts | want_sums << 1 | for_work << 2)})
        mix(w);
    for (size_t j = 0; j < (size_t)n_jobs; ++j) {
        uint64_t w;
        memcpy(&w, jobs + 2 * j, sizeof w);
        mix(w);
    }
    for (size_t i = 0; i < (size_t)n_bins * n_edges; ++i) {
        uint64_t w;
        memcpy(&w, t + i, sizeof w);
        mix(w);
    }
}

struct HostPlan {
    CallKey key;
    uint64_t stamp = 0;
    bool empty = false;
    bool split = false;
    int grid_div = 8;
    int R = 0, band_ne = 0, cap = 0, hp_shift = 0, lean_bins = 0, mode = 0, reach = 0, kernel = 0, nf = 0, n_orient = 0;
    bool band = false, band32 = false, band_fine = false, filter = false, lean = false, merged = false, run_unweighted = false,
         run_weighted = false, strip_items = false, swap = false, sweep = false, triple = false, uni = false, uniform_t = false,
         weighted = false, weighted_any = false;
    int64_t abytes = 0, cand = 0, n_items = 0, n_out = 0, n_pslots = 0, n_sjobs = 0, n_slots = 0, slab = 0, tile = 0;
    double rwin_max = 0.0;
    size_t lds_band = 0, lds_merged = 0;
    unsigned char *d_in = nullptr;
    size_t o_jobs = 0, o_prefix = 0, o_t = 0, o_dthr = 0, o_rwin = 0, o_thr32 = 0, o_tabs = 0, o_cprefix = 0;
    int64_t n_chunks = 0, n_oslots = 0;
    ~HostPlan() { if (d_in) (void)hipFree(d_in); }
};

void drop_plans(yawhip_ctx *ctx, const yawhip_catalog *c) {
    for (size_t i = 0; i < ctx->plans.size();) {
        if (!c || ctx->plans[i]->key.c1_uid == c->uid || ctx->plans[i]->key.c2_uid == c->uid) {
            delete ctx->plans[i];
            ctx->plans[i] = ctx->plans.back();
            ctx->plans.pop_back();
        } else ++i;
    }
}

int check_call(const yawhip_ctx *ctx, const yawhip_catalog *c1, const yawhip_catalog *c2, int32_t n_jobs, const int32_t *jobs,
               int32_t n_bins, int32_t n_edges, const double *t) {
    if (!ctx || !c1 || !c2) return fail(YAWHIP_ERR_INVALID, "yawhip_count_pairs: NULL handle");
    if (n_jobs < 0 || n_bins <= 0 || n_edges < 2 || n_edges > MAX_EDGES || !t || (n_jobs > 0 && !jobs))
        return fail(YAWHIP_ERR_INVALID, "yawhip_count_pairs: bad sizes (n_jobs=%d n_bins=%d n_edges=%d, max edges %d)",
                    n_jobs, n_bins, n_edges, MAX_EDGES);
    if (c1->ctx != ctx || c2->ctx != ctx) return fail(YAWHIP_ERR_MISMATCH, "catalogues belong to another context");
    if (c1->n_patches != c2->n_patches)
        return fail(YAWHIP_ERR_MISMATCH, "patch counts differ (%d vs %d)", c1->n_patches, c2->n_patches);
    return YAWHIP_OK;
}

int make_plan(yawhip_ctx *ctx, const yawhip_catalog *c1, const yawhip_catalog *c2, int32_t n_jobs, const int32_t *jobs,
              int32_t n_bins, int32_t n_edges, const double *t, int32_t kernel, bool want_counts, bool want_sums, bool for_work,
              HostPlan &P) {
    if ((c1->nb != 1 && c1->nb != n_bins) || (c2->nb != 1 && c2->nb != n_bins))
        return fail(YAWHIP_ERR_MISMATCH, "catalogue bin counts (%d, %d) do not fit n_bins=%d", c1->nb, c2->nb, n_bins);
    for (int k = 0; k < n_bins; ++k)
        for (int e = 0; e < n_edges; ++e) {
            const double v = t[(size_t)k * n_edges + e];
            if (!(v >= 0.0) || (e > 0 && !(v >= t[(size_t)k * n_edges + e - 1])))
                return fail(YAWHIP_ERR_INVALID, "thresholds of bin %d are not ascending non-negative numbers", k);
        }
    for (int j = 0; j < n_jobs; ++j)
        if (jobs[2 * j] < 0 || jobs[2 * j] >= c1->n_patches || jobs[2 * j + 1] < 0 || jobs[2 * j + 1] >= c1->n_patches)
            return fail(YAWHIP_ERR_INVALID, "job %d has a patch id outside [0,%d)", j, c1->n_patches);
    if (kernel == YAWHIP_KERNEL_AUTO) kernel = ctx->default_kernel;
    const bool auto_pick = kernel == YAWHIP_KERNEL_AUTO;
    if (kernel == YAWHIP_KERNEL_AUTO) kernel = YAWHIP_KERNEL_BAND;
    if (kernel < YAWHIP_KERNEL_EXACT || kernel > YAWHIP_KERNEL_BAND)
        return fail(YAWHIP_ERR_INVALID, "unknown kernel id %d", kernel);
    const bool unit = c1->unit_norm && c2->unit_norm;
    if (kernel == YAWHIP_KERNEL_FILTER && !unit) kernel = YAWHIP_KERNEL_EXACT;
    if ((kernel == YAWHIP_KERNEL_SWEEP || kernel == YAWHIP_KERNEL_BAND) && c1->axis != c2->axis)
        kernel = unit ? YAWHIP_KERNEL_FILTER : YAWHIP_KERNEL_EXACT;
    if (kernel == YAWHIP_KERNEL_BAND && !unit) kernel = YAWHIP_KERNEL_EXACT;
    bool band = kernel == YAWHIP_KERNEL_BAND;
    const bool sweep = kernel == YAWHIP_KERNEL_SWEEP || band;
    const bool filter = unit && kernel != YAWHIP_KERNEL_EXACT;

    const int nf = n_edges - 1;
    const int64_t n_slots = (int64_t)n_jobs * n_bins;
    const int64_t n_out = n_slots * nf;
    const bool weighted = (c1->w != nullptr) || (c2->w != nullptr);
    P.n_out = n_out;
    if (n_out == 0) { P.empty = true; return YAWHIP_OK; }
    if (n_slots > (1ll << 30)) return fail(YAWHIP_ERR_INVALID, "too many (job,bin) slots");
    HIP_TRY(hipSetDevice(ctx->device));

    const bool weighted_any = (c1->w != nullptr) || (c2->w != nullptr);
    const bool lean = sweep && (filter || band);
    double rwin_max = 0.0;
    for (int k = 0; k < n_bins; ++k)
        rwin_max = std::max(rwin_max, std::sqrt(t[(size_t)k * n_edges + n_edges - 1]) * (1.0 + 1e-12) + 1e-15);
    const bool strips = lean && c1->has_strips && c2->has_strips && c1->strip_width == c2->strip_width &&
                        (c1->strip_width <= 0.0 || rwin_max / c1->strip_width <= (double)MAX_STRIP_REACH);
    bool seg_ok = false;
    if (strips && c1->nb == n_bins && c2->nb == n_bins && n_bins > 1 && ctx->seg_strips) {
        const StripLayout &base2 = c2->strips[c2->axis];
        const int64_t seg_runs = base2.h_vbase[(size_t)base2.n_groups] * (int64_t)c2->nb;
        seg_ok = c2->n / std::max<int64_t>(seg_runs, 1) >= ctx->seg_min_run;
    }
    bool uniform_t = true;
    for (int k = 1; k < n_bins && uniform_t; ++k)
        uniform_t = memcmp(t, t + (size_t)k * n_edges, sizeof(double) * n_edges) == 0;
    const size_t merged_lds = (size_t)n_bins * nf * (weighted_any ? 8 : 4) + (size_t)(uniform_t ? 1 : n_bins) * n_edges * sizeof(double) +
                              (size_t)n_bins * sizeof(float) + BandLds<BCAP_MID>::FIXED + (BCAP_MID + 2) * 8 + 2 * MSTAGE * sizeof(ObjF) + 1024;
    const bool merged_fits = merged_lds <= (size_t)ctx->lds_limit;
    const int mode = !strips ? 0 : (c1->nb > 1 && c2->nb == 1) ? (merged_fits ? 1 : 0) : (seg_ok ? 3 : 0);
    const bool merged = mode == 1;
    const bool strip_items = mode != 0;
    std::vector<int32_t> orient((size_t)n_jobs, (int32_t)c1->axis);
    const StripLayout *L1[3] = {nullptr, nullptr, nullptr}, *L2[3] = {nullptr, nullptr, nullptr};
    if (strip_items) {
        bool need[3] = {false, false, false};
        for (int j = 0; j < n_jobs; ++j) {
            if (ctx->auto_orient) {
                const double *b1 = &c1->h_box[(size_t)6 * jobs[2 * j]], *b2 = &c2->h_box[(size_t)6 * jobs[2 * j + 1]];
                double best = -1.0;
                int wax = (c1->axis + 1) % 3;
                for (int a = 0; a < 3; ++a) {
                    const double m = (b1[a] <= b1[3 + a] ? 0.5 * (b1[a] + b1[3 + a]) : 0.0) +
                                     (b2[a] <= b2[3 + a] ? 0.5 * (b2[a] + b2[3 + a]) : 0.0);
                    if (std::fabs(m) > best) { best = std::fabs(m); wax = a; }
                }
                orient[(size_t)j] = (wax + 2) % 3;
            }
            need[orient[(size_t)j]] = true;
        }
        for (int o = 0; o < 3; ++o) {
            if (!need[o]) continue;
            int rc = build_strip_layout(ctx, const_cast<yawhip_catalog *>(c1), o, mode == 3);
            if (rc == YAWHIP_OK && c2 != c1) rc = build_strip_layout(ctx, const_cast<yawhip_catalog *>(c2), o, mode == 3);
            if (rc != YAWHIP_OK) return rc;
            L1[o] = mode == 3 ? &c1->seg[o] : &c1->strips[o];
            L2[o] = mode == 3 ? &c2->seg[o] : &c2->strips[o];
        }
    }
    const bool want32 = band && strip_items && unit && n_edges <= 4 && ctx->band_fp32 != 0 &&
                        band32_lds(weighted_any, BCAP_MID, (merged ? n_bins : 1) * nf, merged && !uniform_t ? n_bins : 0, n_edges) <=
                            (size_t)ctx->lds_limit;
    std::vector<float> fine32;
    if (band && strip_items && unit && n_edges > 4 && ctx->band_fp32 != 0 &&
        band32_fine_lds(weighted_any, BCAP_MID, (merged ? n_bins : 1) * nf, uniform_t ? 1 : n_bins, n_edges) <= (size_t)ctx->lds_limit)
        fine32 = build_fine32(t, n_bins, n_edges);
    const bool want_fine = !fine32.empty();
    bool swap = (want32 || want_fine) && merged;
    const yawhip_catalog *c_lane = swap ? c1 : c2, *c_strm = swap ? c2 : c1;
    const StripLayout *const *LL = swap ? L1 : L2, *const *LS = swap ? L2 : L1;
    if (auto_pick && band && unit) {
        bool use_sweep = mode == 0;
        if (!use_sweep && !want32 && !want_fine) {
            double obj_run = 0.0;
            for (int o = 0; o < 3; ++o)
                if (LS[o]) obj_run = std::max(obj_run, LS[o]->obj_run);
            use_sweep = obj_run < (double)BAND_MIN_STREAM_RUN;
        }
        if (use_sweep) {
            kernel = YAWHIP_KERNEL_SWEEP;
            band = false;
        }
    }
    const bool band32 = want32 && band, band_fine = want_fine && band;
    if (!band32 && !band_fine && swap) {
        swap = false;
        c_lane = c2; c_strm = c1; LL = L2; LS = L1;
    }
    int R = ctx->tile_r;
    double est_window = 0.0;
    if (R == 0) {
        int64_t max_seg = 0;
        if (strip_items) {
            int64_t n_runs = 1;
            for (int o = 0; o < 3; ++o)
                if (LL[o]) n_runs = std::max(n_runs, LL[o]->h_vbase[(size_t)LL[o]->n_groups]);
            max_seg = c_lane->n / std::max<int64_t>(n_runs, 1);
            if (mode == 3) max_seg = std::max<int64_t>(max_seg, 4 * MWG * 2);
        } else {
            for (int j = 0; j < n_jobs; ++j)
                for (int k = 0; k < (c2->nb == 1 ? 1 : n_bins); ++k) max_seg = std::max(max_seg, seg_len(c2, jobs[2 * j + 1], k));
        }
        const int wg = lean ? MWG : WG;
        R = max_seg >= 8 * wg * 4 ? 4 : (max_seg >= 4 * wg * 2 ? 2 : 1);
        if (strip_items && R > 2) R = 2;
        if (band && strip_items) {
            R = 2;
            auto per_u = [](const auto *c, const StripLayout *const *Ls) {
                int64_t runs = 1;
                for (int o = 0; o < 3; ++o)
                    if (Ls[o]) runs = std::max(runs, Ls[o]->h_vbase[(size_t)Ls[o]->n_groups]);
                double extent = 0.0;
                int n_ext = 0;
                for (int p = 0; p < c->n_patches; ++p) {
                    const double *b = &c->h_box[(size_t)6 * p];
                    double widest = 0.0;
                    for (int a = 0; a < 3; ++a) widest = std::max(widest, b[3 + a] - b[a]);
                    if (widest > 0.0) { extent += widest; ++n_ext; }
                }
                extent = n_ext ? extent / n_ext : 1.0;
                return ((double)c->n / (double)runs) / std::max(extent, 1e-6);
            };
            const double d1 = per_u(c_strm, LS), d2 = per_u(c_lane, LL);
            if (mode == 3 && d1 >= 0.5 * d2) R = 1;
            est_window = 64.0 * R * d1 / std::max(d2, 1e-12) + 2.0 * rwin_max * d1;
        }
    }
    if (band && R == 0) R = 2;
    bool triple = false;
    if ((band32 || band_fine) && strip_items && ctx->triple_runs && c_strm->n < (1ll << 31) && c1->strip_width > 0.0 &&
        (int)std::floor(rwin_max / c1->strip_width + 1e-6) + 1 == 1) {
        const double est3 = 3.0 * est_window;
        triple = ctx->triple_runs == 2 ||
                 (band32 ? est3 <= 0.88 * (B32_CAP_BIG - 4) : est3 <= 0.9 * BCAP_MID);
        for (int o = 0; o < 3 && triple; ++o) {
            if (!LS[o]) continue;
            const int rc = build_triples(ctx, const_cast<yawhip_catalog *>(c_strm), o, mode == 3);
            if (rc == YAWHIP_ERR_OOM) triple = false;
            else if (rc != YAWHIP_OK) return rc;
        }
        if (triple) est_window = est3;
    }
    if (g_trace.on) fprintf(stderr, "[yawhip trace] est_window %.1f (triple %d) R %d mode %d\n", est_window, (int)triple, R, mode);
    int cap = ctx->band_cap == BCAP || ctx->band_cap == BCAP_MID ? ctx->band_cap : 0;
    if (band && cap == 0) cap = R >= 4 || est_window > 0.95 * BCAP ? BCAP_MID : BCAP;
    if (band) {
        if (R == 1) cap = BCAP;
        if (R == 4 && cap == BCAP) cap = BCAP_MID;
    }
    int cap32 = ctx->band_cap == B32_CAP || ctx->band_cap == B32_CAP_BIG ? ctx->band_cap
                                                                         : (est_window > 0.75 * (B32_CAP - 4) ? B32_CAP_BIG : B32_CAP);
    if (R == 1) cap32 = B32_CAP;
    if (R >= 4) cap32 = B32_CAP_BIG;
    if (band32) cap = cap32;
    const int64_t tile = (int64_t)(lean ? MWG : WG) * R;
    const int lean_bins = merged ? n_bins : 1;
    const size_t lds_merged = 2 * MSTAGE * sizeof(ObjF) + (size_t)lean_bins * n_edges * sizeof(double) +
                              (size_t)lean_bins * nf * (weighted_any ? 8 * (MWG / 64) : 4) + (size_t)lean_bins * sizeof(float) +
                              (size_t)MWG * sizeof(unsigned int) + 16;
    int hp_shift = lean_bins * nf <= 32 ? 2 : 0;
    if (band) {
        double coherence = merged ? 0.0 : 1.0;
        if (merged)
            for (int o = 0; o < 3; ++o)
                if (L1[o]) coherence = std::max(coherence, L1[o]->same_bin);
        if (coherence > 0.25) {
            const int cell = weighted_any ? 8 : 4;
            while (hp_shift < (merged ? 3 : 4) && ((size_t)lean_bins * nf * cell << (hp_shift + 1)) <= 2048) ++hp_shift;
        }
    }
    if (ctx->hist_copies_log2 >= 0) hp_shift = ctx->hist_copies_log2;
    const int band_ne = (!merged || uniform_t) && n_edges <= 4 ? n_edges : (nf == 1 ? 2 : 0);
    const bool band_thr = !(band_ne >= 2 && (!merged || uniform_t));
    const size_t LDS_FIXED = (size_t)band_lds_fixed(cap);
    auto band_lds_for = [&](int shift) {
        return band_lds_dynamic(weighted_any, band_thr, lean_bins, n_edges, 1 << shift, cap, merged && !uniform_t ? lean_bins : 1);
    };
    while (band && hp_shift > 0 && band_lds_for(hp_shift) + LDS_FIXED > (size_t)ctx->lds_limit) --hp_shift;
    const size_t lds_band = band_lds_for(hp_shift);
    if (lean && (band ? lds_band + LDS_FIXED : lds_merged) > (size_t)ctx->lds_limit)
        return fail(YAWHIP_ERR_INVALID, "too many bins x edges for the LDS histogram (%zu bytes)", band ? lds_band + LDS_FIXED : lds_merged);

    std::vector<int64_t> prefix;
    std::vector<JobRec> job_recs;
    int64_t n_items = 0, cand = 0, abytes = 0;
    const int obj_bytes1 = c1->w ? 32 : 24, obj_bytes2 = c2->w ? 32 : 24;
    int reach = 0;
    const int tile_idx = R == 1 ? 0 : (R == 2 ? 1 : 2);
    std::vector<int32_t> sjobs;
    const int64_t n_sjobs = mode == 3 ? n_slots : (int64_t)n_jobs;
    const bool half_ok = band32 && triple && R == 1 && c1 == c2 && !swap && ctx->half_bands != 0 && !for_work;
    if (strip_items) {
        const double width = c1->strip_width;
        reach = width > 0.0 ? (int)std::floor(rwin_max / width + 1e-6) + 1 : 0;
        sjobs.resize((size_t)2 * n_sjobs);
        for (int j = 0; j < n_jobs; ++j)
            for (int k = 0; k < (mode == 3 ? n_bins : 1); ++k) {
                const int64_t sj = mode == 3 ? (int64_t)j * n_bins + k : j;
                sjobs[(size_t)2 * sj] = mode == 3 ? jobs[2 * j] * n_bins + k : jobs[2 * j];
                sjobs[(size_t)2 * sj + 1] = mode == 3 ? jobs[2 * j + 1] * n_bins + k : jobs[2 * j + 1];
            }
        prefix.resize((size_t)n_sjobs + 1);
        job_recs.assign((size_t)n_sjobs, JobRec{0, 0, 0, 0, 0});
        for (int64_t j = 0; j < n_sjobs; ++j) {
            const int p = sjobs[(size_t)2 * j + (swap ? 1 : 0)], q = sjobs[(size_t)2 * j + (swap ? 0 : 1)];
            const int o = orient[(size_t)(mode == 3 ? j / n_bins : j)];
            const StripLayout &sl1 = *LS[o], &sl2 = *LL[o];
            const std::vector<int64_t> &tiles = sl2.h_tiles[tile_idx];
            JobRec &jr = job_recs[(size_t)j];
            jr.o = o | (half_ok && p == q ? 4 : 0);
            prefix[(size_t)j] = n_items;
            const int64_t cnt1 = sl1.h_vbase[(size_t)p + 1] - sl1.h_vbase[(size_t)p], lo1 = sl1.h_slo[(size_t)p];
            const int64_t cnt2 = sl2.h_vbase[(size_t)q + 1] - sl2.h_vbase[(size_t)q], lo2 = sl2.h_slo[(size_t)q];
            const int64_t s_lo = std::max<int64_t>(lo1 - reach - lo2, 0), s_hi = std::min<int64_t>(lo1 + cnt1 - 1 + reach - lo2, cnt2 - 1);
            if (cnt1 > 0 && s_hi >= s_lo) {
                const int64_t r0 = sl2.h_vbase[(size_t)q] + s_lo;
                jr.t_lo = tiles[(size_t)r0];
                jr.k_off = lo2 - sl2.h_vbase[(size_t)q] - lo1;
                jr.vbase1 = sl1.h_vbase[(size_t)p];
                jr.n_strips1 = (int32_t)cnt1;
                if (triple) {
                    jr.k_off += 1;
                    jr.vbase1 += 2 * (int64_t)p;
                    jr.n_strips1 += 2;
                }
                n_items += (tiles[(size_t)(r0 + s_hi - s_lo + 1)] - tiles[(size_t)r0]) * ((2 * reach + 1 + MAX_WIN - 1) / MAX_WIN);
            }
        }
        prefix[(size_t)n_sjobs] = n_items;
    } else {
        prefix.resize((size_t)n_slots + 1);
    }
    const int64_t n_pslots = merged ? (int64_t)n_jobs : n_slots;
    auto patch_total = [](const yawhip_catalog *c, int patch) {
        return c->h_off[(size_t)(patch + 1) * c->nb] - c->h_off[(size_t)patch * c->nb];
    };
    for (int j = 0; j < n_jobs; ++j) {
        const int p = jobs[2 * j], q = jobs[2 * j + 1];
        if (strip_items && (c1->nb == 1 || c2->nb == 1)) {
            cand += c1->nb == 1 ? patch_total(c1, p) * patch_total(c2, q) * (c2->nb == 1 ? n_bins : 1)
                                : patch_total(c1, p) * patch_total(c2, q);
        } else {
            for (int k = 0; k < n_bins; ++k) {
                const int64_t n1 = seg_len(c1, p, k), n2 = seg_len(c2, q, k);
                if (!strip_items) prefix[(size_t)j * n_bins + k] = n_items;
                if (n1 > 0 && n2 > 0) {
                    if (!strip_items) n_items += (n2 + tile - 1) / tile;
                    cand += n1 * n2;
                }
            }
        }
        abytes += patch_total(c1, p) * obj_bytes1 + patch_total(c2, q) * obj_bytes2;
    }
    if (!strip_items) prefix[(size_t)n_pslots] = n_items;
    const int64_t slab = merged ? (int64_t)n_bins * nf : nf;

    const bool run_weighted = weighted && want_sums;
    const bool run_unweighted = want_counts || (!weighted && want_sums);

    std::vector<float> dthr((size_t)3 * n_bins);
    auto round_down = [](double v) { float f = (float)v; if ((double)f > v) f = nextafterf(f, -4.0f); return f; };
    for (int k = 0; k < n_bins; ++k) {
        const double thi = t[(size_t)k * n_edges + n_edges - 1];
        float thr32 = ctx->debug_no_hits ? 2.0f : round_down(1.0 - 0.5 * thi - FILTER_GUARD);
        dthr[(size_t)3 * k] = thr32;
        dthr[(size_t)3 * k + 1] = 0.f;
        dthr[(size_t)3 * k + 2] = 0.f;
    }
    std::vector<double> rwin((size_t)n_bins);
    for (int k = 0; k < n_bins; ++k) rwin[(size_t)k] = std::sqrt(t[(size_t)k * n_edges + n_edges - 1]) * (1.0 + 1e-12) + 1e-15;
    if (merged) rwin[0] = rwin_max;
    if (n_jobs > 1 && !for_work &&
        ((run_weighted && n_items * slab * (int64_t)sizeof(double) > ctx->slab_budget) || n_items >= (1ll << 31)))
        { P.split = true; return YAWHIP_OK; }
    DevTab h_tabs[6];
    memset(h_tabs, 0, sizeof h_tabs);
    if (strip_items) {
        for (int o = 0; o < 3; ++o) {
            if (!L1[o]) continue;
            const StripLayout &a = *L1[o], &b = *L2[o];
            h_tabs[o] = make_tab(a.x, a.y, a.z, a.w, merged ? a.k : nullptr, a.off, a.d_vbase, a.d_slo, a.d_tiles[tile_idx],
                                 a.d_tile_rec[tile_idx], a.d_grid, o, a.q, a.q_stride);
            h_tabs[3 + o] = make_tab(b.x, b.y, b.z, b.w, nullptr, b.off, b.d_vbase, b.d_slo, b.d_tiles[tile_idx],
                                     b.d_tile_rec[tile_idx], b.d_grid, o, b.q, b.q_stride);
            if (triple) {
                const StripLayout &st = swap ? b : a;
                DevTab &tb = h_tabs[swap ? 3 + o : o];
                tb = make_tab(st.x, st.y, st.z, st.w3, nullptr, st.off3, st.d_vbase, st.d_slo, st.d_tiles[tile_idx],
                              st.d_tile_rec[tile_idx], st.d_grid3, o, st.q3, st.q3_stride, st.idx3);
                if (half_ok) h_tabs[3 + o].pos3 = (gi32p)b.pos3;
            }
        }
    } else {
        h_tabs[0] = make_tab(c1->x, c1->y, c1->z, c1->w, nullptr, c1->off, nullptr, nullptr, nullptr, nullptr, nullptr, c1->axis);
        h_tabs[3] = make_tab(c2->x, c2->y, c2->z, c2->w, nullptr, c2->off, nullptr, nullptr, nullptr, nullptr, nullptr, c2->axis);
    }
    static_assert(sizeof(JobRec) == 8 * sizeof(int32_t), "JobRec is 32 bytes");
    const size_t n_jobtab = strip_items ? (size_t)8 * n_sjobs : (size_t)2 * n_jobs;
    size_t off_in = 0;
    auto take = [&](size_t bytes) { const size_t o = off_in; off_in = align16(off_in + bytes); return o; };
    const size_t o_jobs = take(n_jobtab * sizeof(int32_t));
    const size_t o_prefix = take(((size_t)n_pslots + 1) * sizeof(int64_t));
    const size_t o_t = take((size_t)n_bins * n_edges * sizeof(double));
    const size_t o_dthr = take((size_t)3 * n_bins * sizeof(float));
    const size_t o_rwin = take((size_t)n_bins * sizeof(double));
    const std::vector<float> thr32 = band32 ? build_thr32(t, n_bins, n_edges) : (band_fine ? fine32 : std::vector<float>());
    const size_t o_thr32 = take(thr32.size() * sizeof(float));
    const size_t o_tabs = take(sizeof h_tabs);
    const int64_t n_oslots = !lean ? n_slots : (merged ? (int64_t)n_jobs : n_slots);
    std::vector<int64_t> cprefix;
    if (run_weighted) {
        cprefix.assign((size_t)n_oslots + 1, 0);
        for (int64_t sl = 0; sl < n_oslots; ++sl)
            cprefix[(size_t)sl + 1] = cprefix[(size_t)sl] + (prefix[(size_t)sl + 1] - prefix[(size_t)sl] + REDUCE_CHUNK - 1) / REDUCE_CHUNK;
    }
    const size_t o_cprefix = take(cprefix.size() * sizeof(int64_t));
    std::vector<unsigned char> image(off_in, 0);
    if (strip_items) {
        memcpy(image.data() + o_jobs, job_recs.data(), sizeof(JobRec) * n_sjobs);
    } else {
        memcpy(image.data() + o_jobs, jobs, sizeof(int32_t) * 2 * n_jobs);
    }
    memcpy(image.data() + o_prefix, prefix.data(), sizeof(int64_t) * ((size_t)n_pslots + 1));
    memcpy(image.data() + o_t, t, sizeof(double) * n_bins * n_edges);
    memcpy(image.data() + o_dthr, dthr.data(), sizeof(float) * 3 * n_bins);
    memcpy(image.data() + o_rwin, rwin.data(), sizeof(double) * n_bins);
    if (!thr32.empty()) memcpy(image.data() + o_thr32, thr32.data(), sizeof(float) * thr32.size());
    memcpy(image.data() + o_tabs, h_tabs, sizeof h_tabs);
    if (!cprefix.empty()) memcpy(image.data() + o_cprefix, cprefix.data(), sizeof(int64_t) * cprefix.size());
    HIP_TRY(hipMalloc(reinterpret_cast<void **>(&P.d_in), std::max<size_t>(off_in, 16)));
    HIP_TRY(hipMemcpy(P.d_in, image.data(), off_in, hipMemcpyHostToDevice));
    P.o_jobs = o_jobs; P.o_prefix = o_prefix; P.o_t = o_t; P.o_dthr = o_dthr; P.o_rwin = o_rwin; P.o_thr32 = o_thr32;
    P.o_tabs = o_tabs; P.o_cprefix = o_cprefix;
    P.n_chunks = cprefix.empty() ? 0 : cprefix.back();
    P.n_oslots = n_oslots;
    P.n_orient = (L1[0] ? 1 : 0) + (L1[1] ? 1 : 0) + (L1[2] ? 1 : 0);
    {
        double skew = 1.0;
        for (const StripLayout *const *LX : {L1, L2})
            for (int o = 0; o < 3; ++o)
                if (LX[o] && LX[o]->built) {
                    const yawhip_catalog *cx = LX == L1 ? c1 : c2;
                    const double runs = (double)std::max<int64_t>(LX[o]->h_vbase[(size_t)LX[o]->n_groups], 1);
                    skew = std::max(skew, LX[o]->obj_run / std::max((double)cx->n / runs, 1.0));
                }
        P.grid_div = ctx->band_grid_div > 0 ? ctx->band_grid_div : (skew > 2.0 ? 4 : (mode == 3 ? 16 : 8));
        if (g_trace.on) fprintf(stderr, "[yawhip trace] run skew %.2f -> grid / %d\n", skew, P.grid_div);
    }
    P.R = R;
    P.abytes = abytes;
    P.band = band;
    P.band32 = band32;
    P.band_fine = band_fine;
    P.band_ne = band_ne;
    P.cand = cand;
    P.cap = cap;
    P.filter = filter;
    P.hp_shift = hp_shift;
    P.lds_band = lds_band;
    P.lds_merged = lds_merged;
    P.lean = lean;
    P.lean_bins = lean_bins;
    P.merged = merged;
    P.mode = mode;
    P.n_items = n_items;
    P.n_out = n_out;
    P.n_pslots = n_pslots;
    P.n_sjobs = n_sjobs;
    P.n_slots = n_slots;
    P.nf = nf;
    P.reach = reach;
    P.run_unweighted = run_unweighted;
    P.run_weighted = run_weighted;
    P.rwin_max = rwin_max;
    P.slab = slab;
    P.strip_items = strip_items;
    P.swap = swap;
    P.sweep = sweep;
    P.tile = tile;
    P.triple = triple;
    P.uniform_t = uniform_t;
    P.uni = merged || band_fine ? uniform_t : true;
    P.weighted = weighted;
    P.weighted_any = weighted_any;
    P.kernel = kernel;
    g_trace.mark("planned");
    return YAWHIP_OK;
}

int count_enqueue(yawhip_ctx *ctx, const yawhip_catalog *c1, const yawhip_catalog *c2, int32_t n_jobs,
                  const int32_t *jobs, int32_t n_bins, int32_t n_edges, const double *t, int32_t kernel,
                  bool want_counts, bool want_sums, int64_t *job_work, CallState &cs, bool fetch_results = true) {
    cs = CallState{};
    cs.wall0 = std::chrono::steady_clock::now();
    g_trace.mark("enqueue");
    cs.want_counts = want_counts;
    cs.want_sums = want_sums;
    HIP_TRY(hipSetDevice(ctx->device));
    CallKey key(ctx, c1, c2, n_jobs, jobs, n_bins, n_edges, t, kernel, want_counts, want_sums, job_work != nullptr);
    HostPlan *plan = nullptr;
    for (HostPlan *cand_plan : ctx->plans)
        if (cand_plan->key == key) {
            plan = cand_plan;
            break;
        }
    if (!plan) {
        std::unique_ptr<HostPlan> fresh(new (std::nothrow) HostPlan());
        if (!fresh) return fail(YAWHIP_ERR_OOM, "host allocation failed");
        const int rc = make_plan(ctx, c1, c2, n_jobs, jobs, n_bins, n_edges, t, kernel, want_counts, want_sums, job_work != nullptr, *fresh);
        if (rc != YAWHIP_OK) return rc;
        key.keep();
        fresh->key = std::move(key);
        if (ctx->plans.size() >= MAX_PLANS) {
            size_t old = 0;
            for (size_t i = 1; i < ctx->plans.size(); ++i)
                if (ctx->plans[i]->stamp < ctx->plans[old]->stamp) old = i;
            HIP_TRY(hipStreamSynchronize(ctx->stream));
            delete ctx->plans[old];
            ctx->plans[old] = ctx->plans.back();
            ctx->plans.pop_back();
        }
        plan = fresh.release();
        ctx->plans.push_back(plan);
    }
    plan->stamp = ++ctx->plan_clock;
    const HostPlan &P = *plan;
    cs.n_out = P.n_out;
    if (P.empty) return YAWHIP_OK;
    if (P.split) return SPLIT_JOBS;
    if (P.run_weighted) HIP_TRY(ctx->d_partials.reserve((size_t)std::max<int64_t>(P.n_items, 1) * P.slab));
    ctx->d_jobs.ptr = reinterpret_cast<int32_t *>(P.d_in + P.o_jobs);
    ctx->d_prefix.ptr = reinterpret_cast<int64_t *>(P.d_in + P.o_prefix);
    ctx->d_t.ptr = reinterpret_cast<double *>(P.d_in + P.o_t);
    ctx->d_dthr.ptr = reinterpret_cast<float *>(P.d_in + P.o_dthr);
    ctx->d_rwin.ptr = reinterpret_cast<double *>(P.d_in + P.o_rwin);
    ctx->d_thr32.ptr = reinterpret_cast<float *>(P.d_in + P.o_thr32);
    ctx->d_tabs.ptr = reinterpret_cast<DevTab *>(P.d_in + P.o_tabs);
    ctx->d_cprefix.ptr = reinterpret_cast<int64_t *>(P.d_in + P.o_cprefix);
    g_trace.mark("plan");
    const size_t o_ctr = 0, o_counts = align16(N_CTR * sizeof(unsigned long long)),
                 o_sums = o_counts + align16((size_t)P.n_out * sizeof(unsigned long long));
    const size_t out_bytes = o_sums + align16((size_t)P.n_out * sizeof(double));
    HIP_TRY(ctx->out.reserve(out_bytes));
    ctx->d_ctr.ptr = reinterpret_cast<unsigned long long *>(ctx->out.d + o_ctr);
    ctx->d_counts.ptr = reinterpret_cast<unsigned long long *>(ctx->out.d + o_counts);
    ctx->d_sums.ptr = reinterpret_cast<double *>(ctx->out.d + o_sums);
    HIP_TRY(hipMemsetAsync(ctx->out.d, 0, P.n_items > 0 ? o_sums : out_bytes, ctx->stream));

    int launches = 0;
    const int64_t n_pot = P.n_items;
    int64_t n_items = P.n_items;
    unsigned long long seg_cap = 0;
    g_trace.mark("memset");
    HIP_TRY(hipEventRecord(ctx->ev0, ctx->stream));
    if (n_pot > 0) {
        if (n_pot >= (1ll << 31))
            return fail(YAWHIP_ERR_INVALID, "too many work items (%lld) in one job", (long long)n_pot);
        const int bwg = build_wg_for(n_pot);
        const unsigned bgrid = (unsigned)((n_pot + bwg - 1) / bwg);
        if (P.strip_items && (P.band32 || P.band_fine) && !job_work && ctx->item_segments)
            seg_cap = (unsigned long long)((bgrid + ITEM_SEGS - 1) / ITEM_SEGS) * (unsigned long long)bwg;
        HIP_TRY(ctx->d_items.reserve(seg_cap ? (size_t)(seg_cap * ITEM_SEGS) : (size_t)n_pot));
        unsigned char *kept_flags = nullptr;
        if (P.run_weighted && P.sweep) {
            HIP_TRY(ctx->d_kept.reserve((size_t)n_pot));
            HIP_TRY(hipMemsetAsync(ctx->d_kept.ptr, 0, (size_t)n_pot, ctx->stream));
            kept_flags = ctx->d_kept.ptr;
        }
        if (P.strip_items)
            hipLaunchKernelGGL(k_build_items_strips, dim3(bgrid), dim3(bwg), 0, ctx->stream, ctx->d_tabs.ptr,
                               reinterpret_cast<const JobRec *>(ctx->d_jobs.ptr), ctx->d_prefix.ptr, (int)P.n_sjobs,
                               P.triple ? 0 : P.reach, (int)P.tile, P.rwin_max, P.swap ? 1 : 0, P.triple ? 1 : 0, n_pot, ctx->d_items.ptr,
                               ctx->d_ctr.ptr, kept_flags, seg_cap);
        else if (P.sweep)
            hipLaunchKernelGGL(k_build_items<true>, dim3(bgrid), dim3(bwg), 0, ctx->stream, view_of(c1), view_of(c2),
                               ctx->d_jobs.ptr, ctx->d_prefix.ptr, (int)P.n_pslots, n_bins, (int)P.tile,
                               ctx->d_rwin.ptr, n_pot, ctx->d_items.ptr, ctx->d_ctr.ptr, kept_flags);
        else
            hipLaunchKernelGGL(k_build_items<false>, dim3(bgrid), dim3(bwg), 0, ctx->stream, view_of(c1), view_of(c2),
                               ctx->d_jobs.ptr, ctx->d_prefix.ptr, (int)P.n_pslots, n_bins, (int)P.tile, ctx->d_rwin.ptr, n_pot,
                               ctx->d_items.ptr, ctx->d_ctr.ptr, nullptr);
        HIP_TRY(hipGetLastError());
        ++launches;
        n_items = n_pot;
        if (P.strip_items && !P.band && n_pot > SYNC_GRID_MIN_ITEMS) {
            HIP_TRY(hipMemcpyAsync(ctx->out.h, ctx->d_ctr.ptr, 2 * sizeof(unsigned long long), hipMemcpyDeviceToHost, ctx->stream));
            HIP_TRY(hipStreamSynchronize(ctx->stream));
            n_items = (int64_t)reinterpret_cast<unsigned long long *>(ctx->out.h)[0];
        }
    }
    if (job_work) {
        HIP_TRY(ctx->d_jobwork.reserve((size_t)n_jobs));
        HIP_TRY(hipMemsetAsync(ctx->d_jobwork.ptr, 0, sizeof(unsigned long long) * (size_t)n_jobs, ctx->stream));
        if (n_pot > 0) {
            hipLaunchKernelGGL(k_item_work, dim3((unsigned)((n_pot + 255) / 256)), dim3(256), 0, ctx->stream, ctx->d_items.ptr,
                               ctx->d_ctr.ptr, P.merged ? 1 : n_bins, ctx->d_jobwork.ptr);
            HIP_TRY(hipGetLastError());
        }
        HIP_TRY(hipMemcpyAsync(job_work, ctx->d_jobwork.ptr, sizeof(int64_t) * (size_t)n_jobs, hipMemcpyDeviceToHost,
                               ctx->stream));
        HIP_TRY(hipStreamSynchronize(ctx->stream));
        return YAWHIP_OK;
    }
    auto reduce_partials = [&](int64_t n_oslots, int64_t values) -> hipError_t {
        const int64_t n_chunks = P.n_chunks;
        if (n_oslots != P.n_oslots) return hipErrorInvalidValue;
        hipError_t er = ctx->d_chunk_sums.reserve((size_t)std::max<int64_t>(n_chunks, 1) * values);
        if (er != hipSuccess) return er;
        const int thr = 256;
        const bool all_kept = !(P.run_weighted && P.sweep);
        if (n_chunks > 0)
            hipLaunchKernelGGL(k_reduce_chunks, dim3((unsigned)((n_chunks * values + thr - 1) / thr)), dim3(thr), 0, ctx->stream,
                               ctx->d_partials.ptr, all_kept ? nullptr : ctx->d_kept.ptr, ctx->d_prefix.ptr, ctx->d_cprefix.ptr,
                               (int)n_oslots, (int)values, ctx->d_chunk_sums.ptr);
        hipLaunchKernelGGL(k_reduce_slots, dim3((unsigned)((n_oslots * values + thr - 1) / thr)), dim3(thr), 0, ctx->stream,
                           ctx->d_chunk_sums.ptr, ctx->d_cprefix.ptr, (int)n_oslots, (int)values, ctx->d_sums.ptr);
        return hipGetLastError();
    };
    HIP_TRY(hipEventRecord(ctx->evc0, ctx->stream));
    int64_t grid = P.strip_items && n_pot > 65536 ? n_pot / P.grid_div : n_pot;
    const int batch_log2 = ctx->band_batch_log2 >= 0 ? ctx->band_batch_log2 : 0;
    if (!P.run_weighted) grid = std::max<int64_t>(grid >> batch_log2, 8);
    grid = std::min<int64_t>((grid + 7) & ~7ll, 1ll << 22);
    const dim3 band_grid((unsigned)grid), wave(64);
    int flush_log2 = ctx->flush_log2;
    while (flush_log2 > 0 && ((uint64_t)64 * P.R * 2 * P.cap << flush_log2) >= (1ull << 32)) --flush_log2;
    const unsigned flush_mask = (1u << flush_log2) - 1u;
    const std::pair<int, int> stage{P.R, P.cap};
    const std::pair<bool, bool> rows{P.merged, P.uni};
    auto launch_band32 = [&](bool wgt) -> hipError_t {
        const size_t lds = band32_lds(P.weighted_any, P.cap, P.lean_bins * P.nf, P.merged && !P.uniform_t ? n_bins : 0, n_edges);
        const bool one_chunk = P.triple || !P.strip_items;
        return pick<Bool<false>, Bool<true>>(wgt, [&](auto w) {
            return pick<Int<4>, Int<3>, Int<2>>(n_edges, [&](auto ne) {
                return pick<Rows<true, false>, Rows<true, true>, Rows<false, true>>(rows, [&](auto r) {
                    return pick<Stage<4, B32_CAP_BIG>, Stage<2, B32_CAP_BIG>, Stage<2, B32_CAP>, Stage<1, B32_CAP>>(stage, [&](auto s) {
                        using S = decltype(s);
                        using M = decltype(r);
                        auto kern = one_chunk ? k_count_band32_one<S::R, S::CAP, w, ne, M::MERGED, M::UNI>
                                              : k_count_band32<S::R, S::CAP, w, ne, M::MERGED, M::UNI>;
                        return launch(kern, band_grid, wave, lds, ctx->stream, ctx->d_tabs.ptr, ctx->d_items.ptr, n_bins, ctx->d_t.ptr,
                                      ctx->d_thr32.ptr, ctx->d_rwin.ptr, flush_mask, P.swap ? 1 : 0, ctx->d_counts.ptr,
                                      ctx->d_partials.ptr, ctx->d_ctr.ptr, seg_cap);
                    });
                });
            });
        });
    };
    auto launch_band64 = [&](bool wgt) -> hipError_t {
        return pick<Bool<false>, Bool<true>>(wgt, [&](auto w) {
            return pick<Int<0>, Int<4>, Int<3>, Int<2>>(P.band_ne, [&](auto ne) {
                return pick<Rows<true, false>, Rows<true, true>, Rows<false, true>>(rows, [&](auto r) {
                    return pick<Stage<4, BCAP_MID>, Stage<2, BCAP_MID>, Stage<2, BCAP>, Stage<1, BCAP>>(stage, [&](auto s) {
                        using S = decltype(s);
                        using M = decltype(r);
                        return launch(k_count_band<S::R, S::CAP, w, ne, M::MERGED, M::UNI>, band_grid, wave, P.lds_band, ctx->stream,
                                      ctx->d_tabs.ptr, ctx->d_items.ptr, n_bins, n_edges, ctx->d_t.ptr, ctx->d_rwin.ptr, flush_mask,
                                      P.hp_shift, w ? 0 : batch_log2, ctx->d_counts.ptr, ctx->d_partials.ptr, ctx->d_ctr.ptr);
                    });
                });
            });
        });
    };
    auto launch_fine = [&](bool wgt) -> hipError_t {
        const size_t lds = band32_fine_lds(P.weighted_any, P.cap, P.lean_bins * P.nf, P.uniform_t ? 1 : n_bins, n_edges);
        return pick<Bool<false>, Bool<true>>(wgt, [&](auto w) {
            return pick<Rows<true, false>, Rows<true, true>, Rows<false, false>, Rows<false, true>>(rows, [&](auto r) {
                return pick<Stage<4, BCAP_MID>, Stage<2, BCAP_MID>, Stage<2, BCAP>, Stage<1, BCAP>>(stage, [&](auto s) {
                    using S = decltype(s);
                    using M = decltype(r);
                    return launch(k_count_band32_fine<S::R, S::CAP, w, M::MERGED, M::UNI>, band_grid, wave, lds, ctx->stream,
                                  ctx->d_tabs.ptr, ctx->d_items.ptr, n_bins, n_edges, ctx->d_t.ptr, ctx->d_thr32.ptr, ctx->d_rwin.ptr,
                                  flush_mask, P.swap ? 1 : 0, ctx->d_counts.ptr, ctx->d_partials.ptr, ctx->d_ctr.ptr, seg_cap);
                });
            });
        });
    };
    auto in_pieces = [&](int wg, auto &&launch_at) -> hipError_t {
        const int64_t max_grid = (1ll << 31) / wg;
        for (int64_t base = 0; base < n_items; base += max_grid) {
            const hipError_t e = launch_at(dim3((unsigned)std::min(max_grid, n_items - base)), base);
            if (e != hipSuccess) return e;
        }
        return hipSuccess;
    };
    auto launch_lean = [&](bool wgt) -> hipError_t {
        return pick<Bool<false>, Bool<true>>(wgt, [&](auto w) {
            return pick<Bool<false>, Bool<true>>(P.nf == 1, [&](auto nf1) {
                return pick<Bool<false>, Bool<true>>(P.merged, [&](auto m) {
                    return pick<Int<4>, Int<2>, Int<1>>(P.R, [&](auto r) {
                        return in_pieces(MWG, [&](dim3 g, int64_t base) {
                            return launch(pick_count_merged<r, w, nf1, m>(), g, dim3(MWG), P.lds_merged, ctx->stream, ctx->d_tabs.ptr,
                                          ctx->d_items.ptr, n_bins, n_edges, ctx->d_t.ptr, ctx->d_dthr.ptr, ctx->d_rwin.ptr, base,
                                          ctx->d_counts.ptr, ctx->d_partials.ptr, ctx->d_ctr.ptr);
                        });
                    });
                });
            });
        });
    };
    const size_t lds_fixed = 2 * STAGE * (sizeof(Obj) + sizeof(ObjF)) + (size_t)((n_edges + 1) & ~1) * sizeof(double);
    auto lds_for = [&](bool w, bool priv) { return lds_fixed + (size_t)P.nf * (priv ? WG : 1) * (w ? 8 : 4); };
    auto launch_plain = [&](bool wgt) -> hipError_t {
        const bool priv = lds_for(wgt, true) <= (size_t)ctx->lds_limit;
        return pick<Bool<true>, Bool<false>>(wgt, [&](auto w) {
            return pick<Bool<false>, Bool<true>>(priv, [&](auto pv) {
                return pick<Bool<false>, Bool<true>>(P.filter, [&](auto f) {
                    return pick<Int<4>, Int<2>, Int<1>>(P.R, [&](auto r) {
                        return in_pieces(WG, [&](dim3 g, int64_t base) {
                            return launch(k_count<r, w, pv, f>, g, dim3(WG), lds_for(w, pv), ctx->stream, view_of(c1), view_of(c2),
                                          ctx->d_items.ptr, n_bins, n_edges, ctx->d_t.ptr, ctx->d_dthr.ptr, base, ctx->d_counts.ptr,
                                          ctx->d_partials.ptr, ctx->d_ctr.ptr);
                        });
                    });
                });
            });
        });
    };
    const bool band_ran = n_items > 0 && P.lean && P.band;
    auto launch_count = [&](bool wgt) {
        if (band_ran) return P.band32 ? launch_band32(wgt) : (P.band_fine ? launch_fine(wgt) : launch_band64(wgt));
        return P.lean ? launch_lean(wgt) : launch_plain(wgt);
    };
    if (n_items > 0 && P.run_unweighted) {
        HIP_TRY(launch_count(false));
        ++launches;
    }
    if (n_items > 0 && P.run_weighted) {
        HIP_TRY(launch_count(true));
        ++launches;
        HIP_TRY(reduce_partials(P.merged ? (int64_t)n_jobs : P.n_slots, P.slab));
        launches += 2;
    }
    HIP_TRY(hipEventRecord(ctx->evc1, ctx->stream));
    if (!P.weighted && want_sums) {
        const int thr = 256;
        hipLaunchKernelGGL(k_counts_to_double, dim3((unsigned)((P.n_out + thr - 1) / thr)), dim3(thr), 0, ctx->stream,
                           ctx->d_counts.ptr, ctx->d_sums.ptr, P.n_out);
        HIP_TRY(hipGetLastError());
        ++launches;
    }
    HIP_TRY(hipEventRecord(ctx->ev1, ctx->stream));
    const size_t fetch = !fetch_results ? o_counts : (want_sums ? out_bytes : (want_counts ? o_sums : o_counts));
    HIP_TRY(hipMemcpyAsync(ctx->out.h, ctx->out.d, fetch, hipMemcpyDeviceToHost, ctx->stream));
    cs.pending = true;
    cs.o_ctr = o_ctr; cs.o_counts = o_counts; cs.o_sums = o_sums;
    cs.band_ran = band_ran; cs.run_unweighted = P.run_unweighted; cs.run_weighted = P.run_weighted;
// ... 716 lines not shown
```

Measured before the change: 26300000 billion.

## Build per-job rotated frame layouts so strip keys align with each patch pair

Adds per-(patch, frame) rotated coordinate layouts. Each patch pair is projected into one of several tilted orthonormal frames (orient_frames=2 gives a (2K+1)^2 grid per axis), and the strip sort key and fp32 coordinates come from that rotated frame instead of a fixed Cartesian axis. The aim is tighter strip and band windows for pairs that sit off-axis, so fewer candidate pairs are tested. In exchange it costs extra layout builds, extra device memory per framed layout, and a widened search radius to absorb rotation rounding error.

```diff
diff --git a/yet_another_wizz_amd/csrc/yawhip.hip b/yet_another_wizz_amd/csrc/yawhip.hip
--- a/yet_another_wizz_amd/csrc/yawhip.hip
+++ b/yet_another_wizz_amd/csrc/yawhip.hip
@@ -19,6 +19,7 @@
 #include <type_traits>
 #include <utility>
 #include <functional>
+#include <iterator>
 #include <vector>
 
 #include "yawhip.h"
@@ -173,10 +174,11 @@
     gf32p qx, qy, qz;
     gi32p idx;
     gi32p pos3;
+    gf64p key;
     int32_t axis;
     int32_t pad_;
 };
-__device__ __forceinline__ gf64p tab_key(const DevTab &t) { return t.axis == 0 ? t.x : (t.axis == 1 ? t.y : t.z); }
+__device__ __forceinline__ gf64p tab_key(const DevTab &t) { return t.key; }
 
 struct TileRec {
     int64_t a0;
@@ -1809,10 +1811,12 @@
 
 inline DevTab make_tab(const double *x, const double *y, const double *z, const double *w, const int32_t *k, const int64_t *off,
                        const int64_t *vbase, const int64_t *slo, const int64_t *tiles, const TileRec *tile_rec, const RunGrid *grid,
-                       int axis, const float *q = nullptr, int64_t q_stride = 0, const int32_t *idx = nullptr) {
+                       int axis, const float *q = nullptr, int64_t q_stride = 0, const int32_t *idx = nullptr,
+                       const double *key = nullptr) {
+    if (!key) key = axis == 0 ? x : (axis == 1 ? y : z);
     return DevTab{(gf64p)x, (gf64p)y, (gf64p)z, (gf64p)w, (gi32p)k, (gi64p)off, (gi64p)vbase, (gi64p)slo, (gi64p)tiles,
                   tile_rec, grid, (gf32p)q, (gf32p)(q ? q + q_stride : nullptr), (gf32p)(q ? q + 2 * q_stride : nullptr), (gi32p)idx,
-                  (gi32p)nullptr, axis, 0};
+                  (gi32p)nullptr, (gf64p)key, axis, 0};
 }
 
 template <typename T>
@@ -1949,6 +1953,7 @@
     int seg_min_run = SEG_STRIPS_MIN_RUN;
     int debug_no_hits = 0;
     int auto_orient = 1;
+    int orient_frames = 2;
     int64_t slab_budget = 1ll << 30;
     int band_grid_div = 0;
     int flush_log2 = 17;
@@ -2009,10 +2014,16 @@
     int64_t *off3 = nullptr;
     RunGrid *d_grid3 = nullptr;
     int64_t n_groups = 0;
+    int64_t n_obj = 0;
+    double *key = nullptr;
+    bool own_key = false;
+    int kcol = 0;
     int64_t device_bytes = 0;
     double obj_run = 0.0;
     double same_bin = 0.0;
     void release() {
+        if (own_key && key) (void)hipFree(key);
+        key = nullptr; own_key = false;
         for (void *ptr : {(void *)x, (void *)y, (void *)z, (void *)w, (void *)k, (void *)q, (void *)off, (void *)d_vbase, (void *)d_slo,
                           (void *)d_tiles[0], (void *)d_tiles[1], (void *)d_tiles[2], (void *)d_tile_rec[0], (void *)d_tile_rec[1],
                           (void *)d_tile_rec[2], (void *)d_grid, (void *)q3, (void *)w3, (void *)idx3, (void *)pos3, (void *)off3, (void *)d_grid3})
@@ -2038,6 +2049,12 @@
     bool unit_norm = true;
     int axis = 2;
     StripLayout strips[3], seg[3];
+    struct Framed {
+        int K = 0;
+        std::vector<int64_t> keys;
+        StripLayout L;
+    };
+    std::vector<std::unique_ptr<Framed>> framed;
     std::vector<yawhip_catalog *> replicas;
     bool has_strips = false;
     double strip_width = 0.0;
@@ -2143,6 +2160,38 @@
     q[2 * stride + i] = (float)z[i];
 }
 
+__device__ __forceinline__ double frame_dot(const double *__restrict__ f, double x, double y, double z) {
+    return __builtin_fma(f[2], z, __builtin_fma(f[1], y, f[0] * x));
+}
+__global__ void k_frame_coords(int64_t n, const int64_t *__restrict__ sub_off, int n_groups, const int64_t *__restrict__ src_off,
+                               const double *__restrict__ frames, const double *__restrict__ x, const double *__restrict__ y,
+                               const double *__restrict__ z, uint32_t *__restrict__ src, double *__restrict__ ku,
+                               double *__restrict__ kv, double *__restrict__ kw) {
+    const int64_t i = (int64_t)blockIdx.x * blockDim.x + threadIdx.x;
+    if (i >= n) return;
+    const int g = segment_of(sub_off, n_groups, i);
+    const int64_t s = src_off[g] + (i - sub_off[g]);
+    const double *f = frames + (size_t)9 * g;
+    const double px = x[s], py = y[s], pz = z[s];
+    src[i] = (uint32_t)s;
+    ku[i] = frame_dot(f, px, py, pz);
+    kv[i] = frame_dot(f + 3, px, py, pz);
+    kw[i] = frame_dot(f + 6, px, py, pz);
+}
+__global__ void k_frame_gather(int64_t n, const uint32_t *__restrict__ perm2, const uint32_t *__restrict__ src,
+                               const double *__restrict__ ku, const double *__restrict__ kv, const double *__restrict__ kw,
+                               uint32_t *__restrict__ perm_cat, double *__restrict__ key, int64_t stride, float *__restrict__ q) {
+    const int64_t i = (int64_t)blockIdx.x * blockDim.x + threadIdx.x;
+    if (i >= n) return;
+    const uint32_t j = perm2[i];
+    perm_cat[i] = src[j];
+    const double u = ku[j];
+    key[i] = u;
+    q[i] = (float)u;
+    q[stride + i] = (float)kv[j];
+    q[2 * stride + i] = (float)kw[j];
+}
+
 __global__ void k_same_bin_neighbours(int64_t n, const int32_t *__restrict__ bins, unsigned long long *__restrict__ out) {
     const int64_t i = (int64_t)blockIdx.x * blockDim.x + threadIdx.x;
     const bool same = i + 1 < n && bins[i] == bins[i + 1];
@@ -2257,22 +2306,46 @@
     return c->h_off[i + 1] - c->h_off[i];
 }
 
+struct LayoutSrc {
+    int64_t n = 0;
+    int n_groups = 0;
+    std::vector<int64_t> h_poff;
+    const double *key = nullptr;
+    const double *strip = nullptr;
+    const uint32_t *src = nullptr;
+    const double *kv = nullptr, *kw = nullptr;
+    int kcol = 0;
+    bool want_bins = false;
+};
+
+int build_layout(yawhip_ctx *ctx, yawhip_catalog *c, StripLayout &L, const LayoutSrc &S);
 int build_strip_layout(yawhip_ctx *ctx, yawhip_catalog *c, int o, bool seg) {
     StripLayout &L = seg ? c->seg[o] : c->strips[o];
     if (L.built) return YAWHIP_OK;
-    const int64_t n = c->n, nseg = (int64_t)c->n_patches * c->nb;
-    const int n_groups = seg ? (int)nseg : c->n_patches;
-    const bool want_bins = !seg && c->nb > 1;
+    LayoutSrc S;
+    S.n = c->n;
+    S.n_groups = seg ? (int)((int64_t)c->n_patches * c->nb) : c->n_patches;
+    S.want_bins = !seg && c->nb > 1;
+    S.h_poff.resize((size_t)S.n_groups + 1);
+    for (int g = 0; g <= S.n_groups; ++g) S.h_poff[(size_t)g] = seg ? c->h_off[(size_t)g] : c->h_off[(size_t)g * c->nb];
+    S.key = key_of(c->x, c->y, c->z, o);
+    S.strip = key_of(c->x, c->y, c->z, (o + 2) % 3);
+    S.kcol = o;
+    return build_layout(ctx, c, L, S);
+}
+
+int build_layout(yawhip_ctx *ctx, yawhip_catalog *c, StripLayout &L, const LayoutSrc &S) {
+    const int64_t n = S.n, nseg = (int64_t)c->n_patches * c->nb;
+    const int n_groups = S.n_groups;
+    const bool want_bins = S.want_bins;
     const double width = c->strip_width;
-    const int saxis = (o + 2) % 3;
-    std::vector<int64_t> h_poff((size_t)n_groups + 1);
-    for (int g = 0; g <= n_groups; ++g) h_poff[(size_t)g] = seg ? c->h_off[(size_t)g] : c->h_off[(size_t)g * c->nb];
+    const std::vector<int64_t> &h_poff = S.h_poff;
     const size_t col = (size_t)std::max<int64_t>(n, 1) * sizeof(double) + 16;
-    uint32_t *perm = nullptr, *perm2 = nullptr, *run = nullptr, *run_sorted = nullptr;
+    uint32_t *perm = nullptr, *perm2 = nullptr, *run = nullptr, *run_sorted = nullptr, *perm_cat = nullptr;
     int32_t *gidx = nullptr, *lohi = nullptr;
     int64_t *poff = nullptr;
     auto bail = [&](hipError_t err, const char *what) {
-        for (void *q : {(void *)perm, (void *)perm2, (void *)run, (void *)run_sorted, (void *)gidx, (void *)lohi, (void *)poff})
+        for (void *q : {(void *)perm, (void *)perm2, (void *)run, (void *)run_sorted, (void *)gidx, (void *)lohi, (void *)poff, (void *)perm_cat})
             if (q) (void)hipFree(q);
         if (err == hipSuccess) return (int)YAWHIP_OK;
         L.release();
@@ -2296,8 +2369,7 @@
         e = hipMemcpyAsync(lohi, h_lohi.data(), (size_t)2 * n_groups * sizeof(int32_t), hipMemcpyHostToDevice, ctx->stream);
     if (e != hipSuccess) return bail(e, "strip tables");
     const unsigned ngrid = (unsigned)((n1 + 255) / 256);
-    hipLaunchKernelGGL(k_strip_index, dim3(ngrid), dim3(256), 0, ctx->stream, n, key_of(c->x, c->y, c->z, saxis), width, poff,
-                       n_groups, gidx, lohi);
+    hipLaunchKernelGGL(k_strip_index, dim3(ngrid), dim3(256), 0, ctx->stream, n, S.strip, width, poff, n_groups, gidx, lohi);
     e = hipMemcpyAsync(h_lohi.data(), lohi, (size_t)2 * n_groups * sizeof(int32_t), hipMemcpyDeviceToHost, ctx->stream);
     if (e == hipSuccess) e = hipStreamSynchronize(ctx->stream);
     if (e != hipSuccess) return bail(e, "strip index");
@@ -2317,7 +2389,7 @@
         e = hipMemcpyAsync(L.d_vbase, vbase.data(), (size_t)(n_groups + 1) * sizeof(int64_t), hipMemcpyHostToDevice, ctx->stream);
     if (e == hipSuccess)
         e = hipMemcpyAsync(L.d_slo, slo.data(), (size_t)n_groups * sizeof(int64_t), hipMemcpyHostToDevice, ctx->stream);
-    if (e == hipSuccess) e = yawsort::sort_segments(ctx->sort_ws, ctx->stream, n, key_of(c->x, c->y, c->z, o), poff, n_groups, perm);
+    if (e == hipSuccess) e = yawsort::sort_segments(ctx->sort_ws, ctx->stream, n, S.key, poff, n_groups, perm);
     if (e != hipSuccess) return bail(e, "group sort");
     hipLaunchKernelGGL(k_run_of, dim3(ngrid), dim3(256), 0, ctx->stream, n, perm, gidx, poff, n_groups, L.d_vbase, L.d_slo, run);
     e = yawsort::sort_runs(ctx->sort_ws, ctx->stream, n, run, perm, run_bits, perm2, run_sorted);
@@ -2332,16 +2404,29 @@
     if (e == hipSuccess) e = hipMalloc(reinterpret_cast<void **>(&L.off), (size_t)(n_runs + 1) * sizeof(int64_t));
     if (e == hipSuccess) e = hipMalloc(reinterpret_cast<void **>(&L.d_grid), (size_t)(n_runs + 1) * sizeof(RunGrid));
     if (e == hipSuccess) e = hipMemsetAsync(L.d_grid, 0, (size_t)(n_runs + 1) * sizeof(RunGrid), ctx->stream);
+    if (e == hipSuccess && S.src) e = hipMalloc(reinterpret_cast<void **>(&L.key), col);
+    if (e == hipSuccess && S.src) e = hipMalloc(reinterpret_cast<void **>(&perm_cat), n1 * sizeof(uint32_t));
     if (e != hipSuccess) return bail(e, "strip layout");
-    hipLaunchKernelGGL(k_gather_columns, dim3(ngrid), dim3(256), 0, ctx->stream, n, perm2, c->x, c->y, c->z, c->w, L.x, L.y, L.z, L.w);
+    L.own_key = S.src != nullptr;
+    L.kcol = S.src ? 0 : S.kcol;
+    const uint32_t *gather = perm2;
+    if (S.src) {
+        hipLaunchKernelGGL(k_frame_gather, dim3(ngrid), dim3(256), 0, ctx->stream, n, perm2, S.src, S.key, S.kv, S.kw, perm_cat, L.key,
+                           L.q_stride, L.q);
+        gather = perm_cat;
+    }
+    hipLaunchKernelGGL(k_gather_columns, dim3(ngrid), dim3(256), 0, ctx->stream, n, gather, c->x, c->y, c->z, c->w, L.x, L.y, L.z, L.w);
     if (want_bins)
-        hipLaunchKernelGGL(k_gather_bins, dim3(ngrid), dim3(256), 0, ctx->stream, n, perm2, c->off, nseg, c->nb, L.k);
-    hipLaunchKernelGGL(k_make_q, dim3(ngrid), dim3(256), 0, ctx->stream, n, L.x, L.y, L.z, L.q_stride, L.q);
+        hipLaunchKernelGGL(k_gather_bins, dim3(ngrid), dim3(256), 0, ctx->stream, n, gather, c->off, nseg, c->nb, L.k);
+    if (!S.src) {
+        L.key = L.kcol == 0 ? L.x : (L.kcol == 1 ? L.y : L.z);
+        hipLaunchKernelGGL(k_make_q, dim3(ngrid), dim3(256), 0, ctx->stream, n, L.x, L.y, L.z, L.q_stride, L.q);
+    }
     hipLaunchKernelGGL(k_run_offsets, dim3((unsigned)((n_runs + 1 + 255) / 256)), dim3(256), 0, ctx->stream, run_sorted, n, n_runs,
                        L.off);
     if (n_runs > 0)
         hipLaunchKernelGGL(k_run_grid<double>, dim3((unsigned)((n_runs * (RUN_GRID + 1) + 255) / 256)), dim3(256), 0, ctx->stream, n_runs,
-                           L.off, o == 0 ? L.x : (o == 1 ? L.y : L.z), L.d_grid);
+                           L.off, L.key, L.d_grid);
     std::vector<int64_t> voff((size_t)n_runs + 1);
     e = hipMemcpyAsync(voff.data(), L.off, (size_t)(n_runs + 1) * sizeof(int64_t), hipMemcpyDeviceToHost, ctx->stream);
     unsigned long long h_same = 0;
@@ -2394,7 +2479,8 @@
     L.h_vbase = std::move(vbase);
     L.h_slo = std::move(slo);
     L.n_groups = n_groups;
-    L.device_bytes = (int64_t)col * (c->w ? 4 : 3) + (want_bins ? n * (int64_t)sizeof(int32_t) : 0) + 3 * L.q_stride * (int64_t)sizeof(float) +
+    L.n_obj = n;
+    L.device_bytes = (int64_t)col * ((c->w ? 4 : 3) + (L.own_key ? 1 : 0)) + (want_bins ? n * (int64_t)sizeof(int32_t) : 0) + 3 * L.q_stride * (int64_t)sizeof(float) +
                      (4 * (n_runs + 1) + 2 * (int64_t)n_groups + 1) * (int64_t)sizeof(int64_t) + (n_runs + 1) * (int64_t)sizeof(RunGrid) +
                      (L.h_tiles[0][(size_t)n_runs] + L.h_tiles[1][(size_t)n_runs] + L.h_tiles[2][(size_t)n_runs]) * (int64_t)sizeof(TileRec);
     c->device_bytes += L.device_bytes;
@@ -2402,12 +2488,11 @@
     return bail(hipSuccess, "");
 }
 
-int build_triples(yawhip_ctx *ctx, yawhip_catalog *c, int o, bool seg) {
-    StripLayout &L = seg ? c->seg[o] : c->strips[o];
+int build_triples(yawhip_ctx *ctx, yawhip_catalog *c, StripLayout &L) {
     if (!L.built) return fail(YAWHIP_ERR_INVALID, "build_triples: layout not built");
     if (L.triples) return YAWHIP_OK;
-    const int64_t n = c->n, G = L.n_groups, V = L.h_vbase[(size_t)G], V3 = V + 2 * G;
-    if (3 * n >= (1ll << 31)) return fail(YAWHIP_ERR_INVALID, "build_triples: catalogue too large for 32-bit entry indices");
+    const int64_t n = L.n_obj, G = L.n_groups, V = L.h_vbase[(size_t)G], V3 = V + 2 * G;
+    if (3 * n >= (1ll << 31)) return fail(YAWHIP_ERR_INVALID, "build_triples: layout too large for 32-bit entry indices");
     std::vector<int64_t> off3((size_t)V3 + 1, 0);
     std::vector<int32_t> run_group((size_t)std::max<int64_t>(V, 1), 0);
     for (int64_t g = 0; g < G; ++g) {
@@ -2440,9 +2525,9 @@
     if (e == hipSuccess) e = hipMemcpyAsync(d_run_group, run_group.data(), run_group.size() * sizeof(int32_t), hipMemcpyHostToDevice, ctx->stream);
     if (e == hipSuccess && n > 0) {
         hipLaunchKernelGGL(k_merge_triples, dim3((unsigned)((n + 255) / 256)), dim3(256), 0, ctx->stream, n, V, L.off, d_run_group,
-                           L.d_vbase, L.off3, o == 0 ? L.x : (o == 1 ? L.y : L.z), L.q, L.q_stride, L.w, L.q3, L.q3_stride, L.w3, L.idx3, L.pos3);
+                           L.d_vbase, L.off3, L.key, L.q, L.q_stride, L.w, L.q3, L.q3_stride, L.w3, L.idx3, L.pos3);
         hipLaunchKernelGGL(k_run_grid<float>, dim3((unsigned)((V3 * (RUN_GRID + 1) + 255) / 256)), dim3(256), 0, ctx->stream, V3, L.off3,
-                           L.q3 + (size_t)o * L.q3_stride, L.d_grid3);
+                           L.q3 + (size_t)L.kcol * L.q3_stride, L.d_grid3);
         e = hipGetLastError();
     }
     if (e == hipSuccess) e = hipStreamSynchronize(ctx->stream);
@@ -2457,6 +2542,97 @@
     L.device_bytes += bytes;
     c->device_bytes += bytes;
     L.triples = true;
+    return YAWHIP_OK;
+}
+
+void frame_of(int o, int ta, int tb, int K, double F[9]) {
+    const int iu = o, iv = (o + 2) % 3, iw = (o + 1) % 3;
+    const double a = K > 0 ? (double)ta / K : 0.0, b = K > 0 ? (double)tb / K : 0.0;
+    double w[3] = {0.0, 0.0, 0.0}, u[3] = {0.0, 0.0, 0.0};
+    w[iw] = 1.0; w[iu] = a; w[iv] = b;
+    const double nw = std::sqrt(1.0 + a * a + b * b);
+    for (double &x : w) x /= nw;
+    u[iu] = 1.0;
+    const double d = w[iu];
+    for (int i = 0; i < 3; ++i) u[i] -= d * w[i];
+    const double nu = std::sqrt(u[0] * u[0] + u[1] * u[1] + u[2] * u[2]);
+    for (double &x : u) x /= nu;
+    const double v[3] = {u[1] * w[2] - u[2] * w[1], u[2] * w[0] - u[0] * w[2], u[0] * w[1] - u[1] * w[0]};
+    for (int i = 0; i < 3; ++i) { F[i] = u[i]; F[3 + i] = v[i]; F[6 + i] = w[i]; }
+}
+inline int frame_id(int o, int ta, int tb, int K) { return (o * (2 * K + 1) + ta + K) * (2 * K + 1) + tb + K; }
+
+int framed_layout(yawhip_ctx *ctx, yawhip_catalog *c, int K, const std::vector<int64_t> &need, yawhip_catalog::Framed **out) {
+    *out = nullptr;
+    const yawhip_catalog::Framed *newest = nullptr;
+    for (auto it = c->framed.rbegin(); it != c->framed.rend(); ++it) {
+        if ((*it)->K != K) continue;
+        if (!newest) newest = it->get();
+        if (std::includes((*it)->keys.begin(), (*it)->keys.end(), need.begin(), need.end())) {
+            *out = it->get();
+            return YAWHIP_OK;
+        }
+    }
+    std::vector<int64_t> keys;
+    if (newest) std::set_union(need.begin(), need.end(), newest->keys.begin(), newest->keys.end(), std::back_inserter(keys));
+    else keys = need;
+    const int P = c->n_patches, side = 2 * K + 1;
+    const int G = (int)keys.size();
+    LayoutSrc S;
+    S.n_groups = G;
+    S.want_bins = c->nb > 1;
+    S.h_poff.assign((size_t)G + 1, 0);
+    std::vector<int64_t> src_off((size_t)std::max(G, 1), 0);
+    std::vector<double> frames((size_t)9 * std::max(G, 1), 0.0);
+    for (int g = 0; g < G; ++g) {
+        const int p = (int)(keys[(size_t)g] % P), f = (int)(keys[(size_t)g] / P);
+        const int64_t first = c->h_off[(size_t)p * c->nb], last = c->h_off[(size_t)(p + 1) * c->nb];
+        S.h_poff[(size_t)g + 1] = S.h_poff[(size_t)g] + (last - first);
+        src_off[(size_t)g] = first;
+        frame_of(f / (side * side), (f / side) % side - K, f % side - K, K, &frames[(size_t)9 * g]);
+    }
+    const int64_t n = S.h_poff[(size_t)G];
+    if (n >= (1ll << 31)) return fail(YAWHIP_ERR_INVALID, "framed layout of %lld objects: more than 32-bit entry indices hold", (long long)n);
+    HIP_TRY(hipSetDevice(ctx->device));
+    const size_t n1 = (size_t)std::max<int64_t>(n, 1);
+    int64_t *d_sub_off = nullptr, *d_src_off = nullptr;
+    double *d_frames = nullptr, *ku = nullptr, *kv = nullptr, *kw = nullptr;
+    uint32_t *src = nullptr;
+    auto release = [&]() {
+        for (void *q : {(void *)d_sub_off, (void *)d_src_off, (void *)d_frames, (void *)ku, (void *)kv, (void *)kw, (void *)src})
+            if (q) (void)hipFree(q);
+    };
+    hipError_t e = hipMalloc(reinterpret_cast<void **>(&d_sub_off), ((size_t)G + 1) * sizeof(int64_t));
+    if (e == hipSuccess) e = hipMalloc(reinterpret_cast<void **>(&d_src_off), src_off.size() * sizeof(int64_t));
+    if (e == hipSuccess) e = hipMalloc(reinterpret_cast<void **>(&d_frames), frames.size() * sizeof(double));
+    if (e == hipSuccess) e = hipMalloc(reinterpret_cast<void **>(&ku), n1 * sizeof(double));
+    if (e == hipSuccess) e = hipMalloc(reinterpret_cast<void **>(&kv), n1 * sizeof(double));
+    if (e == hipSuccess) e = hipMalloc(reinterpret_cast<void **>(&kw), n1 * sizeof(double));
+    if (e == hipSuccess) e = hipMalloc(reinterpret_cast<void **>(&src), n1 * sizeof(uint32_t));
+    if (e == hipSuccess) e = hipMemcpyAsync(d_sub_off, S.h_poff.data(), ((size_t)G + 1) * sizeof(int64_t), hipMemcpyHostToDevice, ctx->stream);
+    if (e == hipSuccess) e = hipMemcpyAsync(d_src_off, src_off.data(), src_off.size() * sizeof(int64_t), hipMemcpyHostToDevice, ctx->stream);
+    if (e == hipSuccess) e = hipMemcpyAsync(d_frames, frames.data(), frames.size() * sizeof(double), hipMemcpyHostToDevice, ctx->stream);
+    if (e == hipSuccess && n > 0) {
+        hipLaunchKernelGGL(k_frame_coords, dim3((unsigned)((n + 255) / 256)), dim3(256), 0, ctx->stream, n, d_sub_off, G, d_src_off,
+                           d_frames, c->x, c->y, c->z, src, ku, kv, kw);
+        e = hipGetLastError();
+    }
+    if (e != hipSuccess) {
+        release();
+        return fail(e == hipErrorOutOfMemory ? YAWHIP_ERR_OOM : YAWHIP_ERR_HIP, "framed layout failed: %s", hipGetErrorString(e));
+    }
+    S.n = n;
+    S.key = ku; S.strip = kv; S.kv = kv; S.kw = kw; S.src = src;
+    std::unique_ptr<yawhip_catalog::Framed> fr(new (std::nothrow) yawhip_catalog::Framed());
+    if (!fr) { release(); return fail(YAWHIP_ERR_OOM, "host allocation failed"); }
+    fr->K = K;
+    fr->keys = std::move(keys);
+    int rc = build_layout(ctx, c, fr->L, S);
+    if (rc == YAWHIP_OK && hipStreamSynchronize(ctx->stream) != hipSuccess) rc = fail(YAWHIP_ERR_HIP, "framed layout: stream failed");
+    release();
+    if (rc != YAWHIP_OK) return rc;
+    c->framed.push_back(std::move(fr));
+    *out = c->framed.back().get();
     return YAWHIP_OK;
 }
 
@@ -2566,6 +2742,9 @@
         flag(&yawhip_ctx::debug_no_hits);
     } else if (!strcmp(key, "auto_orient")) {
         flag(&yawhip_ctx::auto_orient);
+    } else if (!strcmp(key, "orient_frames")) {
+        if (value < 0 || value > 8) return fail(YAWHIP_ERR_INVALID, "orient_frames must be in [0, 8]");
+        number(&yawhip_ctx::orient_frames);
     } else if (!strcmp(key, "slab_budget_bytes")) {
         if (value < 4096) return fail(YAWHIP_ERR_INVALID, "slab_budget_bytes must be >= 4096");
         set = [=](yawhip_ctx &c) { c.slab_budget = value; };
@@ -2738,6 +2917,7 @@
         c->strips[o].release();
         c->seg[o].release();
     }
+    for (auto &f : c->framed) f->L.release();
     delete c;
     return YAWHIP_OK;
 }
@@ -2946,33 +3126,6 @@
     const int mode = !strips ? 0 : (c1->nb > 1 && c2->nb == 1) ? (merged_fits ? 1 : 0) : (seg_ok ? 3 : 0);
     const bool merged = mode == 1;
     const bool strip_items = mode != 0;
-    std::vector<int32_t> orient((size_t)n_jobs, (int32_t)c1->axis);
-    const StripLayout *L1[3] = {nullptr, nullptr, nullptr}, *L2[3] = {nullptr, nullptr, nullptr};
-    if (strip_items) {
-        bool need[3] = {false, false, false};
-        for (int j = 0; j < n_jobs; ++j) {
-            if (ctx->auto_orient) {
-                const double *b1 = &c1->h_box[(size_t)6 * jobs[2 * j]], *b2 = &c2->h_box[(size_t)6 * jobs[2 * j + 1]];
-                double best = -1.0;
-                int wax = (c1->axis + 1) % 3;
-                for (int a = 0; a < 3; ++a) {
-                    const double m = (b1[a] <= b1[3 + a] ? 0.5 * (b1[a] + b1[3 + a]) : 0.0) +
-                                     (b2[a] <= b2[3 + a] ? 0.5 * (b2[a] + b2[3 + a]) : 0.0);
-                    if (std::fabs(m) > best) { best = std::fabs(m); wax = a; }
-                }
-                orient[(size_t)j] = (wax + 2) % 3;
-            }
-            need[orient[(size_t)j]] = true;
-        }
-        for (int o = 0; o < 3; ++o) {
-            if (!need[o]) continue;
-            int rc = build_strip_layout(ctx, const_cast<yawhip_catalog *>(c1), o, mode == 3);
-            if (rc == YAWHIP_OK && c2 != c1) rc = build_strip_layout(ctx, const_cast<yawhip_catalog *>(c2), o, mode == 3);
-            if (rc != YAWHIP_OK) return rc;
-            L1[o] = mode == 3 ? &c1->seg[o] : &c1->strips[o];
-            L2[o] = mode == 3 ? &c2->seg[o] : &c2->strips[o];
-        }
-    }
     const bool want32 = band && strip_items && unit && n_edges <= 4 && ctx->band_fp32 != 0 &&
                         band32_lds(weighted_any, BCAP_MID, (merged ? n_bins : 1) * nf, merged && !uniform_t ? n_bins : 0, n_edges) <=
                             (size_t)ctx->lds_limit;
@@ -2981,6 +3134,87 @@
         band32_fine_lds(weighted_any, BCAP_MID, (merged ? n_bins : 1) * nf, uniform_t ? 1 : n_bins, n_edges) <= (size_t)ctx->lds_limit)
         fine32 = build_fine32(t, n_bins, n_edges);
     const bool want_fine = !fine32.empty();
+    bool frames = strip_items && mode == 1 && (want32 || want_fine) && ctx->auto_orient && ctx->orient_frames > 0;
+    std::vector<int32_t> orient((size_t)n_jobs, (int32_t)c1->axis);
+    const StripLayout *L1[3] = {nullptr, nullptr, nullptr}, *L2[3] = {nullptr, nullptr, nullptr};
+    std::vector<int32_t> fgroup1, fgroup2;
+    int n_orient = 0;
+    if (strip_items) {
+        bool need[3] = {false, false, false};
+        const int K = ctx->orient_frames;
+        std::vector<int64_t> fid(frames ? (size_t)n_jobs : 0);
+        for (int j = 0; j < n_jobs; ++j) {
+            if (ctx->auto_orient) {
+                const double *b1 = &c1->h_box[(size_t)6 * jobs[2 * j]], *b2 = &c2->h_box[(size_t)6 * jobs[2 * j + 1]];
+                double best = -1.0, m[3];
+                int wax = (c1->axis + 1) % 3;
+                for (int a = 0; a < 3; ++a) {
+                    m[a] = (b1[a] <= b1[3 + a] ? 0.5 * (b1[a] + b1[3 + a]) : 0.0) + (b2[a] <= b2[3 + a] ? 0.5 * (b2[a] + b2[3 + a]) : 0.0);
+                    if (std::fabs(m[a]) > best) { best = std::fabs(m[a]); wax = a; }
+                }
+                orient[(size_t)j] = (wax + 2) % 3;
+                if (frames) {
+                    const int o = orient[(size_t)j];
+                    auto step = [&](double num) {
+                        const double r = m[wax] != 0.0 ? num / m[wax] : 0.0;
+                        return (int)std::max<double>(-K, std::min<double>(K, std::nearbyint(r * K)));
+                    };
+                    fid[(size_t)j] = frame_id(o, step(m[o]), step(m[(o + 2) % 3]), K);
+                }
+            }
+            need[orient[(size_t)j]] = true;
+        }
+        std::vector<int64_t> k1, k2, need1, need2;
+        if (frames) {
+            const int64_t P_ = c1->n_patches;
+            k1.resize((size_t)n_jobs);
+            k2.resize((size_t)n_jobs);
+            for (int j = 0; j < n_jobs; ++j) {
+                k1[(size_t)j] = fid[(size_t)j] * P_ + jobs[2 * j];
+                k2[(size_t)j] = fid[(size_t)j] * P_ + jobs[2 * j + 1];
+            }
+            auto uniq = [](std::vector<int64_t> v) { std::sort(v.begin(), v.end()); v.erase(std::unique(v.begin(), v.end()), v.end()); return v; };
+            need1 = uniq(k1);
+            need2 = uniq(k2);
+            if (c1 == c2) {
+                need1.insert(need1.end(), need2.begin(), need2.end());
+                need2 = need1 = uniq(need1);
+            }
+            auto held = [&](const yawhip_catalog *c, const std::vector<int64_t> &keys) {
+                int64_t tot = 0;
+                for (int64_t k : keys) {
+                    const int64_t p = k % P_;
+                    tot += c->h_off[(size_t)(p + 1) * c->nb] - c->h_off[(size_t)p * c->nb];
+                }
+                return tot;
+            };
+            frames = 3 * std::max(held(c1, need1), held(c2, need2)) < (1ll << 31);
+        }
+        if (frames) {
+            yawhip_catalog::Framed *F1 = nullptr, *F2 = nullptr;
+            int rc = framed_layout(ctx, const_cast<yawhip_catalog *>(c1), K, need1, &F1);
+            if (rc == YAWHIP_OK) rc = c2 == c1 ? (F2 = F1, YAWHIP_OK) : framed_layout(ctx, const_cast<yawhip_catalog *>(c2), K, need2, &F2);
+            if (rc != YAWHIP_OK) return rc;
+            fgroup1.resize((size_t)n_jobs);
+            fgroup2.resize((size_t)n_jobs);
+            for (int j = 0; j < n_jobs; ++j) {
+                fgroup1[(size_t)j] = (int32_t)(std::lower_bound(F1->keys.begin(), F1->keys.end(), k1[(size_t)j]) - F1->keys.begin());
+                fgroup2[(size_t)j] = (int32_t)(std::lower_bound(F2->keys.begin(), F2->keys.end(), k2[(size_t)j]) - F2->keys.begin());
+            }
+            L1[0] = &F1->L;
+            L2[0] = &F2->L;
+        } else {
+            for (int o = 0; o < 3; ++o) {
+                if (!need[o]) continue;
+                int rc = build_strip_layout(ctx, const_cast<yawhip_catalog *>(c1), o, mode == 3);
+                if (rc == YAWHIP_OK && c2 != c1) rc = build_strip_layout(ctx, const_cast<yawhip_catalog *>(c2), o, mode == 3);
+                if (rc != YAWHIP_OK) return rc;
+                L1[o] = mode == 3 ? &c1->seg[o] : &c1->strips[o];
+                L2[o] = mode == 3 ? &c2->seg[o] : &c2->strips[o];
+            }
+        }
+        n_orient = (need[0] ? 1 : 0) + (need[1] ? 1 : 0) + (need[2] ? 1 : 0);
+    }
     bool swap = (want32 || want_fine) && merged;
     const yawhip_catalog *c_lane = swap ? c1 : c2, *c_strm = swap ? c2 : c1;
     const StripLayout *const *LL = swap ? L1 : L2, *const *LS = swap ? L2 : L1;
@@ -3007,10 +3241,13 @@
     if (R == 0) {
         int64_t max_seg = 0;
         if (strip_items) {
-            int64_t n_runs = 1;
+            int64_t n_runs = 1, held = c_lane->n;
             for (int o = 0; o < 3; ++o)
-                if (LL[o]) n_runs = std::max(n_runs, LL[o]->h_vbase[(size_t)LL[o]->n_groups]);
-            max_seg = c_lane->n / std::max<int64_t>(n_runs, 1);
+                if (LL[o] && LL[o]->h_vbase[(size_t)LL[o]->n_groups] > n_runs) {
+                    n_runs = LL[o]->h_vbase[(size_t)LL[o]->n_groups];
+                    held = LL[o]->n_obj;
+                }
+            max_seg = held / std::max<int64_t>(n_runs, 1);
             if (mode == 3) max_seg = std::max<int64_t>(max_seg, 4 * MWG * 2);
         } else {
             for (int j = 0; j < n_jobs; ++j)
@@ -3022,9 +3259,12 @@
         if (band && strip_items) {
             R = 2;
             auto per_u = [](const auto *c, const StripLayout *const *Ls) {
-                int64_t runs = 1;
+                int64_t runs = 1, held = c->n;
                 for (int o = 0; o < 3; ++o)
-                    if (Ls[o]) runs = std::max(runs, Ls[o]->h_vbase[(size_t)Ls[o]->n_groups]);
+                    if (Ls[o] && Ls[o]->h_vbase[(size_t)Ls[o]->n_groups] > runs) {
+                        runs = Ls[o]->h_vbase[(size_t)Ls[o]->n_groups];
+                        held = Ls[o]->n_obj;
+                    }
                 double extent = 0.0;
                 int n_ext = 0;
                 for (int p = 0; p < c->n_patches; ++p) {
@@ -3034,7 +3274,7 @@
                     if (widest > 0.0) { extent += widest; ++n_ext; }
                 }
                 extent = n_ext ? extent / n_ext : 1.0;
-                return ((double)c->n / (double)runs) / std::max(extent, 1e-6);
+                return ((double)held / (double)runs) / std::max(extent, 1e-6);
             };
             const double d1 = per_u(c_strm, LS), d2 = per_u(c_lane, LL);
             if (mode == 3 && d1 >= 0.5 * d2) R = 1;
@@ -3050,7 +3290,7 @@
                  (band32 ? est3 <= 0.88 * (B32_CAP_BIG - 4) : est3 <= 0.9 * BCAP_MID);
         for (int o = 0; o < 3 && triple; ++o) {
             if (!LS[o]) continue;
-            const int rc = build_triples(ctx, const_cast<yawhip_catalog *>(c_strm), o, mode == 3);
+            const int rc = build_triples(ctx, const_cast<yawhip_catalog *>(c_strm), *const_cast<StripLayout *>(LS[o]));
             if (rc == YAWHIP_ERR_OOM) triple = false;
             else if (rc != YAWHIP_OK) return rc;
         }
@@ -3118,12 +3358,13 @@
         prefix.resize((size_t)n_sjobs + 1);
         job_recs.assign((size_t)n_sjobs, JobRec{0, 0, 0, 0, 0});
         for (int64_t j = 0; j < n_sjobs; ++j) {
-            const int p = sjobs[(size_t)2 * j + (swap ? 1 : 0)], q = sjobs[(size_t)2 * j + (swap ? 0 : 1)];
-            const int o = orient[(size_t)(mode == 3 ? j / n_bins : j)];
+            const int pp = sjobs[(size_t)2 * j + (swap ? 1 : 0)], qq = sjobs[(size_t)2 * j + (swap ? 0 : 1)];
+            const int o = frames ? 0 : orient[(size_t)(mode == 3 ? j / n_bins : j)];
             const StripLayout &sl1 = *LS[o], &sl2 = *LL[o];
+            const int p = frames ? (swap ? fgroup2 : fgroup1)[(size_t)j] : pp, q = frames ? (swap ? fgroup1 : fgroup2)[(size_t)j] : qq;
             const std::vector<int64_t> &tiles = sl2.h_tiles[tile_idx];
             JobRec &jr = job_recs[(size_t)j];
-            jr.o = o | (half_ok && p == q ? 4 : 0);
+            jr.o = o | (half_ok && pp == qq ? 4 : 0);
             prefix[(size_t)j] = n_items;
             const int64_t cnt1 = sl1.h_vbase[(size_t)p + 1] - sl1.h_vbase[(size_t)p], lo1 = sl1.h_slo[(size_t)p];
             const int64_t cnt2 = sl2.h_vbase[(size_t)q + 1] - sl2.h_vbase[(size_t)q], lo2 = sl2.h_slo[(size_t)q];
@@ -3185,6 +3426,8 @@
     std::vector<double> rwin((size_t)n_bins);
     for (int k = 0; k < n_bins; ++k) rwin[(size_t)k] = std::sqrt(t[(size_t)k * n_edges + n_edges - 1]) * (1.0 + 1e-12) + 1e-15;
     if (merged) rwin[0] = rwin_max;
+    if (frames)
+        for (double &r : rwin) r += 1e-14;
     if (n_jobs > 1 && !for_work &&
         ((run_weighted && n_items * slab * (int64_t)sizeof(double) > ctx->slab_budget) || n_items >= (1ll << 31)))
         { P.split = true; return YAWHIP_OK; }
@@ -3195,14 +3438,14 @@
             if (!L1[o]) continue;
             const StripLayout &a = *L1[o], &b = *L2[o];
             h_tabs[o] = make_tab(a.x, a.y, a.z, a.w, merged ? a.k : nullptr, a.off, a.d_vbase, a.d_slo, a.d_tiles[tile_idx],
-                                 a.d_tile_rec[tile_idx], a.d_grid, o, a.q, a.q_stride);
+                                 a.d_tile_rec[tile_idx], a.d_grid, a.kcol, a.q, a.q_stride, nullptr, a.key);
             h_tabs[3 + o] = make_tab(b.x, b.y, b.z, b.w, nullptr, b.off, b.d_vbase, b.d_slo, b.d_tiles[tile_idx],
-                                     b.d_tile_rec[tile_idx], b.d_grid, o, b.q, b.q_stride);
+                                     b.d_tile_rec[tile_idx], b.d_grid, b.kcol, b.q, b.q_stride, nullptr, b.key);
             if (triple) {
                 const StripLayout &st = swap ? b : a;
                 DevTab &tb = h_tabs[swap ? 3 + o : o];
                 tb = make_tab(st.x, st.y, st.z, st.w3, nullptr, st.off3, st.d_vbase, st.d_slo, st.d_tiles[tile_idx],
-                              st.d_tile_rec[tile_idx], st.d_grid3, o, st.q3, st.q3_stride, st.idx3);
+                              st.d_tile_rec[tile_idx], st.d_grid3, st.kcol, st.q3, st.q3_stride, st.idx3);
                 if (half_ok) h_tabs[3 + o].pos3 = (gi32p)b.pos3;
             }
         }
@@ -3249,15 +3492,14 @@
     P.o_tabs = o_tabs; P.o_cprefix = o_cprefix;
     P.n_chunks = cprefix.empty() ? 0 : cprefix.back();
     P.n_oslots = n_oslots;
-    P.n_orient = (L1[0] ? 1 : 0) + (L1[1] ? 1 : 0) + (L1[2] ? 1 : 0);
+    P.n_orient = n_orient;
     {
         double skew = 1.0;
         for (const StripLayout *const *LX : {L1, L2})
             for (int o = 0; o < 3; ++o)
                 if (LX[o] && LX[o]->built) {
-                    const yawhip_catalog *cx = LX == L1 ? c1 : c2;
                     const double runs = (double)std::max<int64_t>(LX[o]->h_vbase[(size_t)LX[o]->n_groups], 1);
-                    skew = std::max(skew, LX[o]->obj_run / std::max((double)cx->n / runs, 1.0));
+                    skew = std::max(skew, LX[o]->obj_run / std::max((double)LX[o]->n_obj / runs, 1.0));
                 }
         P.grid_div = ctx->band_grid_div > 0 ? ctx->band_grid_div : (skew > 2.0 ? 4 : (mode == 3 ? 16 : 8));
         if (g_trace.on) fprintf(stderr, "[yawhip trace] run skew %.2f -> grid / %d\n", skew, P.grid_div);
```

Result: faster. 27410000 billion (median of 6 runs) (+4.2%).
